# ksahlin/NGSpeciesID

Measured on AMD Instinct MI355X. Metric: reads/sec end-to-end (cluster + spoa consensus + racon x3), 750 bp ONT, higher is better.
Workload: dtype u8 / int16 / int32 DP, 64-bit bit-vectors (f64 thresholds)

## Files before the change

### ngspeciesid_amd/csrc/k_poa.h

```cpp
#pragma once
#include "ngsid_internal.h"

struct PSeq { const uint8_t* s; const uint8_t* q; int32_t len, uw; uint32_t cw; int32_t mode, a0, a1; };

#define POA_MODE_SUBGRAPH 3

struct PoaJobSet {
    const PSeq* seqs; const PSeq* bbs; const uint32_t* seq_idx; const uint32_t* job_off; const int32_t* job_bb; uint32_t njobs; const uint32_t* job_list; uint32_t nrun;
    const uint8_t* job_final;
    const uint32_t* nrun_dev;
    int m, n, g, Vcap, Ecap, Lmax, D, node_cap, trim_tiles;
    int32_t* Hglob; uint8_t* dirglob; uint32_t* covglob;
    uint8_t* out; int32_t* out_len; int32_t* out_span ; uint64_t* out_cw; uint32_t* out_n; uint32_t* out_cov; uint32_t* dropped; uint32_t* slot_overflow; unsigned long long* phase_cycles; int phase_detail; unsigned long long* stat_rows ;
};

__host__ __device__ inline uint32_t poa_ntiles(uint32_t n, uint32_t D) { if (n == 0) return 0; if (D == 0 || n <= D) return 1; const uint32_t r = n % D; return (r != 0 && r < (D + 1) / 2) ? n / D : (n + D - 1) / D; }

struct PoaPlan { int Vcap, Ecap, Lmax; uint32_t nwg_main, nwg_redo; int band0; bool sub = false; };
int32_t poa_check_limits(ngsid_ctx* ctx, const PoaPlan& P, int m, int g);
int32_t poa_prepare(ngsid_ctx* ctx, PoaPlan& P, uint32_t max_jobs, int m, int g);
int32_t poa_launch(ngsid_ctx* ctx, const PoaPlan& P, PoaJobSet J, int band, bool redo, uint32_t* work_ctr, bool sub = false);
```

### ngspeciesid_amd/csrc/ngsid_api.hip

```cpp
#include "ngsid_internal.h"
#include "../../include/ngsid_merge_schedule.h"
#include "../../include/ngsid_tables.h"
#include <math.h>
#include <algorithm>

extern "C" uint32_t ngsid_abi_version(void) { return 2u; }

static char g_static_err[256] = "";
extern "C" const char* ngsid_last_error(ngsid_ctx* ctx) { return ctx ? ctx->err : g_static_err; }

namespace {
struct DevPool { std::mutex mu; std::multimap<unsigned long long, void*> free_; size_t cached = 0; int contexts = 0; size_t live = 0, peak = 0;
                 struct Upload { size_t bs; void* q; size_t bq; void* off; size_t bo; }; std::map<void*, Upload> uploads;
};
DevPool g_pool;
const size_t POOL_LIMIT = (size_t)48 << 30;
const size_t POOL_HEADROOM = (size_t)3 << 30;
struct PoolBlocks { void* p[3] = {nullptr, nullptr, nullptr}; size_t b[3] = {0, 0, 0}; bool owned = true; ~PoolBlocks() { if (owned) for (int i = 0; i < 3; ++i) if (p[i]) ngsid_pool_free(p[i], b[i]); } };
inline size_t pool_class(size_t b) { if (b < 4096) return 4096; int sh = 63 - __builtin_clzll((unsigned long long)b) - 3; size_t m = ((size_t)1 << sh) - 1; return (b + m) & ~m; }
inline unsigned long long pool_key(int dev, size_t cls) { return ((unsigned long long)dev << 56) | (unsigned long long)cls; }
}
thread_local ngsid_ctx* g_ngsid_tls_ctx = nullptr;
hipError_t ngsid_pool_alloc(void** p, size_t bytes, size_t* got)
{
    const size_t cls = pool_class(bytes ? bytes : 1); int dev = 0; (void)hipGetDevice(&dev);
    {
        std::lock_guard<std::mutex> lk(g_pool.mu);
        auto it = g_pool.free_.find(pool_key(dev, cls));
        if (it != g_pool.free_.end()) { *p = it->second; g_pool.free_.erase(it); g_pool.cached -= cls; *got = cls; g_pool.live += cls; g_pool.peak = std::max(g_pool.peak, g_pool.live); return hipSuccess; }
    }
    hipError_t e = hipErrorOutOfMemory;
    for (int attempt = 0; attempt < 2; ++attempt) {
        size_t freeb = 0, totalb = 0;
        const bool known = hipMemGetInfo(&freeb, &totalb) == hipSuccess;
        if (!known || freeb >= cls + std::min<size_t>(POOL_HEADROOM, totalb / 16)) { e = hipMalloc(p, cls); if (e == hipSuccess) break; (void)hipGetLastError(); }
        if (attempt == 0) ngsid_pool_release_all();
    }
    *got = e == hipSuccess ? cls : 0;
    if (e == hipSuccess) { std::lock_guard<std::mutex> lk(g_pool.mu); g_pool.live += cls; g_pool.peak = std::max(g_pool.peak, g_pool.live); }
    return e;
}
void ngsid_pool_free(void* p, size_t bytes)
{
    if (!p) return;
    if (ngsid_ctx* c = g_ngsid_tls_ctx) {
        (void)hipStreamSynchronize(c->stream);
        if (c->ev_fork) for (int i = 0; i < 4; ++i) if (c->side[i]) (void)hipStreamSynchronize(c->side[i]);
    } else (void)hipDeviceSynchronize();
    int dev = 0; (void)hipGetDevice(&dev);
    {
        std::lock_guard<std::mutex> lk(g_pool.mu);
        g_pool.live -= std::min(g_pool.live, bytes);
        if (bytes && g_pool.cached + bytes <= POOL_LIMIT) { g_pool.free_.emplace(pool_key(dev, bytes), p); g_pool.cached += bytes; return; }
    }
    (void)hipFree(p);
}
namespace { struct PinPool { std::mutex mu; std::multimap<size_t, void*> free_; size_t cached = 0; }; PinPool g_pin; const size_t PIN_LIMIT = (size_t)4 << 30; }
void* ngsid_pinned_alloc(size_t bytes)
{
    const size_t cls = pool_class(bytes ? bytes : 1);
    {
        std::lock_guard<std::mutex> lk(g_pin.mu);
        auto it = g_pin.free_.find(cls);
        if (it != g_pin.free_.end()) { void* p = it->second; g_pin.free_.erase(it); g_pin.cached -= cls; return p; }
    }
    void* p = nullptr;
    if (hipHostMalloc(&p, cls, hipHostMallocDefault) != hipSuccess) {
        (void)hipGetLastError();
        std::vector<void*> old; { std::lock_guard<std::mutex> lk(g_pin.mu); for (auto& kv : g_pin.free_) old.push_back(kv.second); g_pin.free_.clear(); g_pin.cached = 0; }
        for (void* q : old) (void)hipHostFree(q);
        if (hipHostMalloc(&p, cls, hipHostMallocDefault) != hipSuccess) { (void)hipGetLastError(); return nullptr; }
    }
    return p;
}
void ngsid_pinned_free(void* p, size_t bytes)
{
    if (!p) return;
    const size_t cls = pool_class(bytes ? bytes : 1);
    {
        std::lock_guard<std::mutex> lk(g_pin.mu);
        if (g_pin.cached + cls <= PIN_LIMIT) { g_pin.free_.emplace(cls, p); g_pin.cached += cls; return; }
    }
    (void)hipHostFree(p);
}
size_t ngsid_pool_cached_bytes() { std::lock_guard<std::mutex> lk(g_pool.mu); return g_pool.cached; }
int ngsid_pool_contexts() { std::lock_guard<std::mutex> lk(g_pool.mu); return g_pool.contexts > 0 ? g_pool.contexts : 1; }
void ngsid_pool_stats(size_t* live, size_t* peak, bool reset_peak) { std::lock_guard<std::mutex> lk(g_pool.mu); if (live) *live = g_pool.live; if (peak) *peak = g_pool.peak; if (reset_peak) g_pool.peak = g_pool.live; }
void ngsid_pool_release_all()
{
    std::lock_guard<std::mutex> lk(g_pool.mu);
    for (auto& kv : g_pool.free_) (void)hipFree(kv.second);
    g_pool.free_.clear(); g_pool.cached = 0;
}

extern "C" int32_t ngsid_create(int32_t device_ordinal, uint32_t flags, ngsid_ctx** out)
{
    (void)flags;
    if (!out) return NGSID_ERR_ARG;
    *out = nullptr;
    int ndev = 0;
    hipError_t e = hipGetDeviceCount(&ndev);
    if (e != hipSuccess || ndev <= 0) { snprintf(g_static_err, sizeof g_static_err, "no HIP device (%s); this library has no CPU path", hipGetErrorString(e)); return NGSID_ERR_NO_DEVICE; }
    if (device_ordinal < 0 || device_ordinal >= ndev) { snprintf(g_static_err, sizeof g_static_err, "device ordinal %d out of range (0..%d)", device_ordinal, ndev - 1); return NGSID_ERR_ARG; }
    e = hipSetDevice(device_ordinal);
    if (e != hipSuccess) { snprintf(g_static_err, sizeof g_static_err, "hipSetDevice: %s", hipGetErrorString(e)); return NGSID_ERR_HIP; }
    ngsid_ctx* c = new ngsid_ctx();
    c->device = device_ordinal;
    c->debug_sync = getenv("NGSID_DEBUG_SYNC") != nullptr;
    hipDeviceProp_t prop;
    if (hipGetDeviceProperties(&prop, device_ordinal) == hipSuccess) {
        c->n_cu = prop.multiProcessorCount > 0 ? prop.multiProcessorCount : 256;
        size_t freeb = 0, totalb = 0;
        if (hipMemGetInfo(&freeb, &totalb) == hipSuccess && freeb > ((size_t)8 << 30)) c->scratch_budget = std::min<size_t>(freeb / 4, (size_t)32 << 30);
    }
    e = hipStreamCreateWithFlags(&c->stream, hipStreamNonBlocking);
    if (e != hipSuccess) { snprintf(g_static_err, sizeof g_static_err, "hipStreamCreate: %s", hipGetErrorString(e)); delete c; return NGSID_ERR_HIP; }
    { std::lock_guard<std::mutex> lk(g_pool.mu); g_pool.contexts++; }
    *out = c;
    return NGSID_OK;
}

extern "C" void ngsid_destroy(ngsid_ctx* ctx)
{
    if (!ctx) return;
    if (g_ngsid_tls_ctx == ctx) g_ngsid_tls_ctx = nullptr;
    (void)hipSetDevice(ctx->device);
    for (int i = 0; i < 4; ++i) { if (ctx->side[i]) { (void)hipStreamSynchronize(ctx->side[i]); (void)hipStreamDestroy(ctx->side[i]); } if (ctx->ev_join[i]) (void)hipEventDestroy(ctx->ev_join[i]); }
    if (ctx->ev_fork) (void)hipEventDestroy(ctx->ev_fork);
    if (ctx->pin) (void)hipHostFree(ctx->pin);
    if (ctx->stream) { (void)hipStreamSynchronize(ctx->stream); (void)hipStreamDestroy(ctx->stream); }
    delete ctx;
    bool last; { std::lock_guard<std::mutex> lk(g_pool.mu); last = --g_pool.contexts <= 0; }
    if (last) {
        {
            std::lock_guard<std::mutex> lk(g_pool.mu);
            for (auto& kv : g_pool.uploads) { (void)hipFree(kv.first); if (kv.second.q) (void)hipFree(kv.second.q); (void)hipFree(kv.second.off); }
            g_pool.uploads.clear();
        }
        ngsid_pool_release_all();
        std::vector<void*> pins; { std::lock_guard<std::mutex> lk(g_pin.mu); for (auto& kv : g_pin.free_) pins.push_back(kv.second); g_pin.free_.clear(); g_pin.cached = 0; }
        for (void* q : pins) (void)hipHostFree(q);
    }
}

int32_t ngsid_side_streams(ngsid_ctx* ctx)
{
    if (ctx->ev_fork) return NGSID_OK;
    for (int i = 0; i < 4; ++i) { HIPCHK(ctx, hipStreamCreateWithFlags(&ctx->side[i], hipStreamNonBlocking)); HIPCHK(ctx, hipEventCreateWithFlags(&ctx->ev_join[i], hipEventDisableTiming)); }
    HIPCHK(ctx, hipEventCreateWithFlags(&ctx->ev_fork, hipEventDisableTiming));
    return NGSID_OK;
}

__global__ __launch_bounds__(256) void k_off_fingerprint(const uint64_t* __restrict__ off, uint64_t n, unsigned long long* __restrict__ out)
{
    unsigned long long h = 0;
    for (uint64_t i = (uint64_t)blockIdx.x * 256 + threadIdx.x; i <= n; i += (uint64_t)gridDim.x * 256) { unsigned long long x = off[i] + (i + 1) * 0xD6E8FEB86659FD93ull; x ^= x >> 31; x *= 0x9E3779B97F4A7C15ull; x ^= x >> 29; h += x; }
#pragma unroll
    for (int d = 32; d >= 1; d >>= 1) h += __shfl_xor(h, d);
    if ((threadIdx.x & 63) == 0) atomicAdd(out, h);
}

int32_t ngsid_upload_reads(ngsid_ctx* ctx, const ngsid_reads_t* in, DevReads* out, bool need_qual)
{
    if (!in || (!in->off) || (in->n && !in->seq)) NGSID_FAIL(ctx, NGSID_ERR_ARG, "null read set");
    if (need_qual && in->n && !in->qual) NGSID_FAIL(ctx, NGSID_ERR_ARG, "this entry point needs qualities");
    HIPCHK(ctx, hipSetDevice(ctx->device));
    HostTimer hu(ctx->stream, "upload_reads");
    out->n = in->n;
    if (in->mem == NGSID_MEM_DEVICE) {
        out->seq = in->seq; out->qual = in->qual; out->off = in->off;
        unsigned long long fp = 0;
        {
            if (ctx->mzc_fp.n < 2) HIPCHK(ctx, ctx->mzc_fp.alloc(2));
            HIPCHK(ctx, hipMemsetAsync(ctx->mzc_fp.p + 1, 0, sizeof(unsigned long long), ctx->stream));
            hipLaunchKernelGGL(k_off_fingerprint, dim3(256), dim3(256), 0, ctx->stream, in->off, in->n, ctx->mzc_fp.p + 1);
            HIPCHK(ctx, hipGetLastError());
            HIPCHK(ctx, hipMemcpyAsync(&fp, ctx->mzc_fp.p + 1, sizeof fp, hipMemcpyDeviceToHost, ctx->stream));
            HIPCHK(ctx, hipStreamSynchronize(ctx->stream));
        }
        if (ctx->offc.v && ctx->offc.ptr == (const void*)in->off && ctx->offc.n == in->n && ctx->offc.fp == fp && ctx->offc.v->size() == in->n + 1) {
            out->h_off.v = ctx->offc.v; out->total = (*out->h_off.v)[in->n]; out->maxlen = ctx->offc.maxlen; out->minlen = ctx->offc.minlen;
            hu.mark("offsets: cached");
            return NGSID_OK;
        }
        out->h_off.resize(in->n + 1);
        hu.mark("resize");
        const size_t nb = sizeof(uint64_t) * (in->n + 1);
        if (ctx->pin_bytes < nb) { if (ctx->pin) (void)hipHostFree(ctx->pin); ctx->pin = nullptr; ctx->pin_bytes = 0; HIPCHK(ctx, hipHostMalloc(&ctx->pin, nb + nb / 8, hipHostMallocDefault)); ctx->pin_bytes = nb + nb / 8; }
        HIPCHK(ctx, hipMemcpyAsync(ctx->pin, in->off, nb, hipMemcpyDeviceToHost, ctx->stream));
        HIPCHK(ctx, hipStreamSynchronize(ctx->stream));
        hu.mark("d2h");
        memcpy(out->h_off.data(), ctx->pin, nb);
        hu.mark("memcpy");
        ctx->offc.ptr = in->off; ctx->offc.n = in->n; ctx->offc.fp = fp; ctx->offc.v = out->h_off.v; ctx->offc.maxlen = 0;
    } else {
        out->h_off.resize(in->n + 1);
        memcpy(out->h_off.data(), in->off, sizeof(uint64_t) * (in->n + 1));
        const uint64_t total = out->h_off[in->n];
        HIPCHK(ctx, out->own_seq.alloc(total + 16)); HIPCHK(ctx, out->own_off.alloc(in->n + 1));
        if (total) HIPCHK(ctx, hipMemcpyAsync(out->own_seq.p, in->seq, total, hipMemcpyHostToDevice, ctx->stream));
        HIPCHK(ctx, hipMemcpyAsync(out->own_off.p, in->off, sizeof(uint64_t) * (in->n + 1), hipMemcpyHostToDevice, ctx->stream));
        out->seq = out->own_seq.p; out->off = out->own_off.p; out->qual = nullptr;
        if (in->qual) { HIPCHK(ctx, out->own_qual.alloc(total + 16)); if (total) HIPCHK(ctx, hipMemcpyAsync(out->own_qual.p, in->qual, total, hipMemcpyHostToDevice, ctx->stream)); out->qual = out->own_qual.p; }
        HIPCHK(ctx, hipStreamSynchronize(ctx->stream));
    }
    out->total = out->h_off[in->n];
    uint32_t mx = 0, mn = 0xffffffffu;
    for (uint64_t i = 0; i < in->n; ++i) {
        if (out->h_off[i + 1] < out->h_off[i]) NGSID_FAIL(ctx, NGSID_ERR_ARG, "offsets not monotone at read %llu", (unsigned long long)i);
        const uint64_t l = out->h_off[i + 1] - out->h_off[i];
        if (l > 0xffffffffull) NGSID_FAIL(ctx, NGSID_ERR_TOO_LONG, "read %llu too long", (unsigned long long)i);
        mx = std::max<uint32_t>(mx, (uint32_t)l); mn = std::min<uint32_t>(mn, (uint32_t)l);
    }
    out->maxlen = mx; out->minlen = in->n ? mn : 0;
    if (in->mem == NGSID_MEM_DEVICE && ctx->offc.v == out->h_off.v) { ctx->offc.maxlen = out->maxlen; ctx->offc.minlen = out->minlen; }
    hu.mark("scan");
    return NGSID_OK;
}

extern "C" int32_t ngsid_sg_align_cigar_batch(ngsid_ctx* ctx, const ngsid_reads_t* queries, const ngsid_reads_t* targets,
                                              const uint32_t* q_idx, const uint32_t* t_idx, uint64_t n_pairs,
                                              int32_t match, int32_t mismatch, const int32_t* open, int32_t ext,
                                              int32_t* score, uint64_t* ops_off, uint8_t* ops, uint64_t cap, uint64_t* needed)
{
    if (!ctx) return NGSID_ERR_ARG;
    if (!queries || !targets || !ops_off || (n_pairs && (!q_idx || !t_idx || !open))) NGSID_FAIL(ctx, NGSID_ERR_ARG, "null argument");
    DevReads Q, T;
    int32_t rc = ngsid_upload_reads(ctx, queries, &Q, false); if (rc) return rc;
    rc = ngsid_upload_reads(ctx, targets, &T, false); if (rc) return rc;
    ops_off[0] = 0;
    if (n_pairs == 0) { if (needed) *needed = 0; return NGSID_OK; }
    uint32_t mq = 0, mt = 0;
    std::vector<uint64_t> h_off(n_pairs + 1, 0);
    for (uint64_t p = 0; p < n_pairs; ++p) {
        if (q_idx[p] >= Q.n || t_idx[p] >= T.n) NGSID_FAIL(ctx, NGSID_ERR_ARG, "pair %llu out of range", (unsigned long long)p);
        const uint32_t ql = (uint32_t)(Q.h_off[q_idx[p] + 1] - Q.h_off[q_idx[p]]), tl = (uint32_t)(T.h_off[t_idx[p] + 1] - T.h_off[t_idx[p]]);
        mq = std::max(mq, ql); mt = std::max(mt, tl);
        h_off[p + 1] = h_off[p] + ql + tl;
    }
    DevBuf<uint32_t> dq, dt; DevBuf<int32_t> dopen, dout; DevBuf<uint64_t> doff; DevBuf<uint8_t> dops;
    HIPCHK(ctx, dq.alloc(n_pairs)); HIPCHK(ctx, dt.alloc(n_pairs)); HIPCHK(ctx, dopen.alloc(n_pairs)); HIPCHK(ctx, dout.alloc(n_pairs * 4)); HIPCHK(ctx, doff.alloc(n_pairs + 1)); HIPCHK(ctx, dops.alloc(h_off[n_pairs] + 1));
    HIPCHK(ctx, hipMemcpyAsync(dq.p, q_idx, 4 * n_pairs, hipMemcpyHostToDevice, ctx->stream));
    HIPCHK(ctx, hipMemcpyAsync(dt.p, t_idx, 4 * n_pairs, hipMemcpyHostToDevice, ctx->stream));
    HIPCHK(ctx, hipMemcpyAsync(dopen.p, open, 4 * n_pairs, hipMemcpyHostToDevice, ctx->stream));
    HIPCHK(ctx, hipMemcpyAsync(doff.p, h_off.data(), 8 * (n_pairs + 1), hipMemcpyHostToDevice, ctx->stream));
    AlignJob J{};
    J.qseq = Q.seq; J.qoff = Q.off; J.tseq = T.seq; J.toff = T.off; J.qidx = dq.p; J.tidx = dt.p; J.npairs = n_pairs;
    J.match = match; J.mismatch = mismatch; J.ext = ext; J.k = 1; J.open = dopen.p; J.match_id = nullptr;
    J.score = dout.p; J.ncols = dout.p + n_pairs; J.nmatch = nullptr; J.region = nullptr; J.bp = nullptr; J.bp_windows = 0; J.window = 1; J.span = nullptr;
    J.ops = dops.p; J.ops_off = doff.p;
    int mo = 0; for (uint64_t p = 0; p < n_pairs; ++p) { if (open[p] < 0) { mo = 1 << 20; break; } mo = std::max(mo, (int)open[p]); }
    rc = ngsid_launch_align(ctx, J, mq, mt, mo); if (rc) return rc;
    std::vector<int32_t> h(n_pairs * 2); std::vector<uint8_t> hops(h_off[n_pairs] + 1);
    HIPCHK(ctx, hipMemcpyAsync(h.data(), dout.p, 8 * n_pairs, hipMemcpyDeviceToHost, ctx->stream));
    HIPCHK(ctx, hipMemcpyAsync(hops.data(), dops.p, h_off[n_pairs], hipMemcpyDeviceToHost, ctx->stream));
    HIPCHK(ctx, hipStreamSynchronize(ctx->stream));
    if (score) memcpy(score, h.data(), 4 * n_pairs);
    uint64_t total = 0; for (uint64_t p = 0; p < n_pairs; ++p) { total += (uint64_t)h[n_pairs + p]; ops_off[p + 1] = total; }
    if (needed) *needed = total;
    if (total > cap || (!ops && total)) NGSID_FAIL(ctx, NGSID_ERR_CAPACITY, "ops buffer too small: need %llu bytes", (unsigned long long)total);
    static const uint8_t sym[4] = {'=', 'X', 'I', 'D'};
    for (uint64_t p = 0; p < n_pairs; ++p) {
        const uint64_t c = (uint64_t)h[n_pairs + p]; const uint8_t* src = hops.data() + h_off[p]; uint8_t* dst = ops + ops_off[p];
        const uint64_t ql = Q.h_off[q_idx[p] + 1] - Q.h_off[q_idx[p]], tl = T.h_off[t_idx[p] + 1] - T.h_off[t_idx[p]];
        if (ql == 0 || tl == 0) { for (uint64_t x = 0; x < c; ++x) dst[x] = ql ? 'I' : 'D'; continue; }
        for (uint64_t x = 0; x < c; ++x) dst[x] = sym[src[c - 1 - x] & 3];
    }
    return NGSID_OK;
}

extern "C" int32_t ngsid_sg_align_batch(ngsid_ctx* ctx, const ngsid_reads_t* queries, const ngsid_reads_t* targets,
                                        const uint32_t* q_idx, const uint32_t* t_idx, uint64_t n_pairs,
                                        int32_t match, int32_t mismatch, const int32_t* open, int32_t ext,
                                        int32_t k, const int32_t* match_id,
                                        int32_t* score, int32_t* n_cols, int32_t* n_match, int32_t* region)
{
    ApiClock api_clock_(ctx, "sg_align_batch");
    if (!ctx) return NGSID_ERR_ARG;
    if (!queries || !targets || (n_pairs && (!q_idx || !t_idx || !open))) NGSID_FAIL(ctx, NGSID_ERR_ARG, "null argument");
    DevReads Q, T;
    int32_t rc = ngsid_upload_reads(ctx, queries, &Q, false); if (rc) return rc;
    rc = ngsid_upload_reads(ctx, targets, &T, false); if (rc) return rc;
    if (n_pairs == 0) return NGSID_OK;
    uint32_t mq = 0, mt = 0;
    for (uint64_t p = 0; p < n_pairs; ++p) {
        if (q_idx[p] >= Q.n || t_idx[p] >= T.n) NGSID_FAIL(ctx, NGSID_ERR_ARG, "pair %llu out of range", (unsigned long long)p);
        mq = std::max<uint32_t>(mq, (uint32_t)(Q.h_off[q_idx[p] + 1] - Q.h_off[q_idx[p]]));
        mt = std::max<uint32_t>(mt, (uint32_t)(T.h_off[t_idx[p] + 1] - T.h_off[t_idx[p]]));
    }
    DevBuf<uint32_t> dq, dt; DevBuf<int32_t> dopen, dmid, dout;
    HIPCHK(ctx, dq.alloc(n_pairs)); HIPCHK(ctx, dt.alloc(n_pairs)); HIPCHK(ctx, dopen.alloc(n_pairs)); HIPCHK(ctx, dmid.alloc(n_pairs)); HIPCHK(ctx, dout.alloc(n_pairs * 4));
    HIPCHK(ctx, hipMemcpyAsync(dq.p, q_idx, 4 * n_pairs, hipMemcpyHostToDevice, ctx->stream));
    HIPCHK(ctx, hipMemcpyAsync(dt.p, t_idx, 4 * n_pairs, hipMemcpyHostToDevice, ctx->stream));
    HIPCHK(ctx, hipMemcpyAsync(dopen.p, open, 4 * n_pairs, hipMemcpyHostToDevice, ctx->stream));
    if (match_id) HIPCHK(ctx, hipMemcpyAsync(dmid.p, match_id, 4 * n_pairs, hipMemcpyHostToDevice, ctx->stream));
    AlignJob J{};
    J.qseq = Q.seq; J.qoff = Q.off; J.tseq = T.seq; J.toff = T.off; J.qidx = dq.p; J.tidx = dt.p; J.npairs = n_pairs;
    J.match = match; J.mismatch = mismatch; J.ext = ext; J.k = k; J.open = dopen.p; J.match_id = match_id ? dmid.p : nullptr;
    J.score = dout.p; J.ncols = dout.p + n_pairs; J.nmatch = dout.p + 2 * n_pairs; J.region = dout.p + 3 * n_pairs;
    J.bp = nullptr; J.bp_windows = 0; J.window = 1; J.span = nullptr;
    int mo = 0; for (uint64_t p = 0; p < n_pairs; ++p) { if (open[p] < 0) { mo = 1 << 20; break; } mo = std::max(mo, (int)open[p]); }
    rc = ngsid_launch_align(ctx, J, mq, mt, mo); if (rc) return rc;
    std::vector<int32_t> h(n_pairs * 4);
    HIPCHK(ctx, hipMemcpyAsync(h.data(), dout.p, 16 * n_pairs, hipMemcpyDeviceToHost, ctx->stream));
    HIPCHK(ctx, hipStreamSynchronize(ctx->stream));
    if (score) memcpy(score, h.data(), 4 * n_pairs);
    if (n_cols) memcpy(n_cols, h.data() + n_pairs, 4 * n_pairs);
    if (n_match) memcpy(n_match, h.data() + 2 * n_pairs, 4 * n_pairs);
    if (region) memcpy(region, h.data() + 3 * n_pairs, 4 * n_pairs);
    return NGSID_OK;
}

extern "C" int32_t ngsid_ed_align_batch(ngsid_ctx* ctx, const ngsid_reads_t* queries, const ngsid_reads_t* targets,
                                        const uint32_t* q_idx, const uint32_t* t_idx, uint64_t n_pairs,
                                        int32_t window, int32_t bp_windows, int32_t* distance, int32_t* span, int32_t* bp)
{
    if (!ctx) return NGSID_ERR_ARG;
    if (!queries || !targets || (n_pairs && (!q_idx || !t_idx))) NGSID_FAIL(ctx, NGSID_ERR_ARG, "null argument");
    if (bp && (bp_windows <= 0 || window <= 0)) NGSID_FAIL(ctx, NGSID_ERR_ARG, "bp needs window > 0 and bp_windows > 0");
    DevReads Q, T;
    int32_t rc = ngsid_upload_reads(ctx, queries, &Q, false); if (rc) return rc;
    rc = ngsid_upload_reads(ctx, targets, &T, false); if (rc) return rc;
    if (n_pairs == 0) return NGSID_OK;
    uint32_t mq = 0, mt = 0;
    for (uint64_t p = 0; p < n_pairs; ++p) {
        if (q_idx[p] >= Q.n || t_idx[p] >= T.n) NGSID_FAIL(ctx, NGSID_ERR_ARG, "pair %llu out of range", (unsigned long long)p);
        mq = std::max<uint32_t>(mq, (uint32_t)(Q.h_off[q_idx[p] + 1] - Q.h_off[q_idx[p]]));
        mt = std::max<uint32_t>(mt, (uint32_t)(T.h_off[t_idx[p] + 1] - T.h_off[t_idx[p]]));
    }
    DevBuf<uint32_t> dq, dt; DevBuf<int32_t> ddist, dspan, dbp;
    HIPCHK(ctx, dq.alloc(n_pairs)); HIPCHK(ctx, dt.alloc(n_pairs)); HIPCHK(ctx, ddist.alloc(n_pairs)); HIPCHK(ctx, dspan.alloc(n_pairs * 4));
    if (bp) HIPCHK(ctx, dbp.alloc(n_pairs * (uint64_t)bp_windows * 4));
    HIPCHK(ctx, hipMemcpyAsync(dq.p, q_idx, 4 * n_pairs, hipMemcpyHostToDevice, ctx->stream));
    HIPCHK(ctx, hipMemcpyAsync(dt.p, t_idx, 4 * n_pairs, hipMemcpyHostToDevice, ctx->stream));
    AlignJob J{};
    J.qseq = Q.seq; J.qoff = Q.off; J.tseq = T.seq; J.toff = T.off; J.qidx = dq.p; J.tidx = dt.p; J.npairs = n_pairs;
    J.bp = bp ? dbp.p : nullptr; J.bp_windows = bp ? bp_windows : 0; J.window = window; J.span = dspan.p;
    rc = ngsid_launch_ed_align(ctx, J, mq, mt, ddist.p); if (rc) return rc;
    if (distance) HIPCHK(ctx, hipMemcpyAsync(distance, ddist.p, 4 * n_pairs, hipMemcpyDeviceToHost, ctx->stream));
    if (span) HIPCHK(ctx, hipMemcpyAsync(span, dspan.p, 16 * n_pairs, hipMemcpyDeviceToHost, ctx->stream));
    if (bp) HIPCHK(ctx, hipMemcpyAsync(bp, dbp.p, 16ull * n_pairs * bp_windows, hipMemcpyDeviceToHost, ctx->stream));
    HIPCHK(ctx, hipStreamSynchronize(ctx->stream));
    return NGSID_OK;
}

extern "C" int32_t ngsid_hpc_minimizers(ngsid_ctx* ctx, const ngsid_reads_t* reads, int32_t k, int32_t w,
                                        uint64_t* mz_off, uint64_t* codes, uint32_t* pos, uint64_t cap, uint64_t* needed,
                                        uint32_t* hpc_len, double* hpc_err)
{
    if (!ctx) return NGSID_ERR_ARG;
    if (!reads || !mz_off) NGSID_FAIL(ctx, NGSID_ERR_ARG, "null argument");
    DevReads R; int32_t rc = ngsid_upload_reads(ctx, reads, &R, false); if (rc) return rc;
    const uint64_t n = R.n;
    DevBuf<uint64_t> ccode, coff; DevBuf<uint32_t> cpos, dcnt, dhl; DevBuf<double> dherr, draw; PinVec<uint64_t> hmoff; PinVec<uint32_t> hcnt(n), hhl(n);
    HIPCHK(ctx, dcnt.alloc(n)); HIPCHK(ctx, dhl.alloc(n)); HIPCHK(ctx, dherr.alloc(n)); HIPCHK(ctx, draw.alloc(n));
    long long bad = -1;
    rc = ngsid_minimizers_csr(ctx, R, k, w, MzOut{&ccode, &cpos, &coff, &hmoff}, dcnt.p, dhl.p, dherr.p, draw.p, hcnt.data(), hhl.data(), &bad); if (rc) return rc;
    if (bad >= 0) NGSID_FAIL(ctx, NGSID_ERR_ALPHABET, "read %lld: base outside ACGTN", bad);
    std::vector<double> hherr(n);
    if (n) HIPCHK(ctx, hipMemcpyAsync(hherr.data(), dherr.p, 8 * n, hipMemcpyDeviceToHost, ctx->stream));
    HIPCHK(ctx, hipStreamSynchronize(ctx->stream));
    const uint64_t total = hmoff[n];
    if (needed) *needed = total;
    if (hpc_len) memcpy(hpc_len, hhl.data(), 4 * n);
    if (hpc_err) memcpy(hpc_err, hherr.data(), 8 * n);
    const bool dev_out = reads->mem == NGSID_MEM_DEVICE;
    if (total > cap || (total && (!codes || !pos))) {
        if (!dev_out) memcpy(mz_off, hmoff.data(), 8 * (n + 1));
        NGSID_FAIL(ctx, NGSID_ERR_CAPACITY, "minimizer buffer too small: need %llu entries", (unsigned long long)total);
    }
    const hipMemcpyKind kind = dev_out ? hipMemcpyDeviceToDevice : hipMemcpyDeviceToHost;
    if (dev_out) HIPCHK(ctx, hipMemcpyAsync(mz_off, coff.p, 8 * (n + 1), kind, ctx->stream)); else memcpy(mz_off, hmoff.data(), 8 * (n + 1));
    if (total) { HIPCHK(ctx, hipMemcpyAsync(codes, ccode.p, 8 * total, kind, ctx->stream)); HIPCHK(ctx, hipMemcpyAsync(pos, cpos.p, 4 * total, kind, ctx->stream)); }
    HIPCHK(ctx, hipStreamSynchronize(ctx->stream));
    return NGSID_OK;
}

__constant__ double c_p_clamped[128];
__constant__ double c_p_nomin[128];
static bool g_score_tables[16] = {false};

#define SC_QS 132
#define SC_SS 68
template <typename HT>
__global__ __launch_bounds__(64)
void k_score_reads(const uint8_t* __restrict__ seq, const uint8_t* __restrict__ qual, const uint64_t* __restrict__ off, uint64_t n,
                   int k, double qthr, double* __restrict__ score, double* __restrict__ err, uint8_t* __restrict__ keep)
{
    __shared__ __attribute__((aligned(16))) uint8_t qt[64 * SC_QS];
    __shared__ __attribute__((aligned(16))) uint8_t st[64 * SC_SS];
    __shared__ HT hist[128 * 64];
    __shared__ double tp[128], tn[128];
    const int lane = threadIdx.x;
    const uint64_t r = (uint64_t)blockIdx.x * 64 + lane;
    const bool have = r < n;
    const uint64_t b = have ? off[r] : 0; const int len = have ? (int)(off[r + 1] - b) : 0;
    tp[lane] = c_p_clamped[lane]; tp[lane + 64] = c_p_clamped[lane + 64]; tn[lane] = c_p_nomin[lane]; tn[lane + 64] = c_p_nomin[lane + 64];
    for (int c = 0; c < 128; ++c) hist[c * 64 + lane] = 0;
    int maxlen = len;
#pragma unroll
    for (int d = 32; d >= 1; d >>= 1) maxlen = max(maxlen, __shfl_xor(maxlen, d));
    maxlen = __builtin_amdgcn_readfirstlane(maxlen);
    const bool active = have && len >= 2 * k;
    int hl = 0; uint8_t prevc = 0;
    double cur = 1.0, sum = 0.0;
    const int sub = lane >> 4, dj = lane & 15;
    for (int c0 = 0; c0 < maxlen; c0 += 64) {
        const int half = c0 & 64;
        for (int it = 0; it < 16; ++it) {
            const int rr = it * 4 + sub;
            const uint64_t rb = __shfl((unsigned long long)b, rr); const int rl = __shfl(len, rr);
            const int x = c0 + dj * 4;
            unsigned qw = 0, sw = 0;
            if (x + 3 < rl) { qw = *(const unsigned*)(qual + rb + x); sw = *(const unsigned*)(seq + rb + x); }
            else for (int y = 0; y < 4; ++y) if (x + y < rl) { qw |= (unsigned)qual[rb + x + y] << (8 * y); sw |= (unsigned)seq[rb + x + y] << (8 * y); }
            *(unsigned*)(qt + rr * SC_QS + half + dj * 4) = qw;
            *(unsigned*)(st + rr * SC_SS + dj * 4) = sw;
        }
        __syncthreads();
        if (active) {
            const int e = min(64, len - c0);
            for (int i = 0; i < e; ++i) {
                const int gi = c0 + i;
                const uint8_t sc = st[lane * SC_SS + i], qc = qt[lane * SC_QS + half + i] & 127;
                hl += (gi == 0 || sc != prevc); prevc = sc;
                hist[qc * 64 + lane] += 1;
                const double pn = 1.0 - tp[qc];
                if (gi < k) { cur = cur * pn; if (gi == k - 1) sum = cur; }
                else { const double leave = 1.0 - tp[qt[lane * SC_QS + ((gi - k) & 127)] & 127]; cur *= (pn / leave); sum += cur; }
            }
        }
        __syncthreads();
    }
    if (!have) return;
    score[r] = 0.0; err[r] = 0.0; keep[r] = 0;
    if (!active || hl < k) return;
    const double ee = (double)(len - k + 1) - sum;
    const double pno = 1.0 - ee / (double)(len - k + 1);
    score[r] = pno * (double)(len - k + 1);
    double se = 0.0;
    for (int c = 0; c < 128; ++c) { const int h = hist[c * 64 + lane]; if (h) se = se + (double)h * tn[c]; }
    const double er = se / (double)len;
    err[r] = er;
    if (10.0 * -(log(er) / log(10.0)) <= qthr) return;
    keep[r] = 1;
}

extern "C" int32_t ngsid_score_reads(ngsid_ctx* ctx, const ngsid_reads_t* reads, int32_t k, double q_threshold,
                                     double* score, double* err_rate, uint8_t* keep)
{
    if (!ctx) return NGSID_ERR_ARG;
    if (!reads || !score || !err_rate || !keep || k < 1) NGSID_FAIL(ctx, NGSID_ERR_ARG, "null argument");
    if (k > 64) NGSID_FAIL(ctx, NGSID_ERR_ARG, "score_reads: k = %d exceeds 64 (the quality ring of the kernel)", (int)k);
    DevReads R; int32_t rc = ngsid_upload_reads(ctx, reads, &R, true); if (rc) return rc;
    if (!g_score_tables[ctx->device & 15]) {
        HIPCHK(ctx, hipMemcpyToSymbol(HIP_SYMBOL(c_p_clamped), NGSID_PHRED_P, sizeof(double) * 128));
        HIPCHK(ctx, hipMemcpyToSymbol(HIP_SYMBOL(c_p_nomin), NGSID_PHRED_P_NOMIN, sizeof(double) * 128));
        g_score_tables[ctx->device & 15] = true;
    }
    const uint64_t n = R.n; if (!n) return NGSID_OK;
    DevBuf<double> ds, de; DevBuf<uint8_t> dk;
    HIPCHK(ctx, ds.alloc(n)); HIPCHK(ctx, de.alloc(n)); HIPCHK(ctx, dk.alloc(n));
    { ProfScope ps_(ctx, "k_score_reads");
      if (R.maxlen <= 65535u) hipLaunchKernelGGL(k_score_reads<unsigned short>, dim3((unsigned)((n + 63) / 64)), dim3(64), 0, ctx->stream, R.seq, R.qual, R.off, n, k, q_threshold, ds.p, de.p, dk.p);
      else hipLaunchKernelGGL(k_score_reads<unsigned int>, dim3((unsigned)((n + 63) / 64)), dim3(64), 0, ctx->stream, R.seq, R.qual, R.off, n, k, q_threshold, ds.p, de.p, dk.p); }
    HIPCHK(ctx, hipGetLastError());
    HIPCHK(ctx, hipMemcpyAsync(score, ds.p, 8 * n, hipMemcpyDeviceToHost, ctx->stream));
    HIPCHK(ctx, hipMemcpyAsync(err_rate, de.p, 8 * n, hipMemcpyDeviceToHost, ctx->stream));
    HIPCHK(ctx, hipMemcpyAsync(keep, dk.p, n, hipMemcpyDeviceToHost, ctx->stream));
    HIPCHK(ctx, hipStreamSynchronize(ctx->stream));
    return NGSID_OK;
}

static void prof_collect(ngsid_ctx* ctx)
{
    (void)hipStreamSynchronize(ctx->stream);
    for (auto& e : ctx->prof_events) {
        float ms = 0.f;
        if (hipEventElapsedTime(&ms, e.a, e.b) == hipSuccess) { auto& acc = ctx->prof_acc[e.name]; acc.first += ms; acc.second += 1; }
        (void)hipEventDestroy(e.a); (void)hipEventDestroy(e.b);
    }
    ctx->prof_events.clear();
}
extern "C" int32_t ngsid_profile_enable(ngsid_ctx* ctx, int32_t on)
{
    if (!ctx) return NGSID_ERR_ARG;
    prof_collect(ctx); ctx->prof_acc.clear(); ctx->prof = on != 0;
    if (on) { if (ctx->stat.n < 8) HIPCHK(ctx, ctx->stat.alloc(8)); HIPCHK(ctx, hipMemsetAsync(ctx->stat.p, 0, 8 * sizeof(unsigned long long), ctx->stream)); HIPCHK(ctx, hipStreamSynchronize(ctx->stream)); }
    return NGSID_OK;
}
extern "C" int32_t ngsid_reads_upload(ngsid_ctx* ctx, const ngsid_reads_t* host, ngsid_reads_t* dev)
{
    if (!ctx) return NGSID_ERR_ARG;
    if (!host || !dev || !host->off || (host->n && !host->seq) || host->mem != NGSID_MEM_HOST) NGSID_FAIL(ctx, NGSID_ERR_ARG, "reads_upload: a host read set and an output are required");
    HIPCHK(ctx, hipSetDevice(ctx->device));
    const uint64_t n = host->n, total = host->off[n];
    PoolBlocks PB; void *&ds = PB.p[0], *&dq = PB.p[1], *&dof = PB.p[2]; size_t &bs = PB.b[0], &bq = PB.b[1], &bo = PB.b[2];
    HIPCHK(ctx, ngsid_pool_alloc(&ds, total + 16, &bs));
    HIPCHK(ctx, ngsid_pool_alloc(&dof, sizeof(uint64_t) * (n + 1), &bo));
    if (host->qual) HIPCHK(ctx, ngsid_pool_alloc(&dq, total + 16, &bq));
    if (total) HIPCHK(ctx, hipMemcpyAsync(ds, host->seq, total, hipMemcpyHostToDevice, ctx->stream));
    if (total && host->qual) HIPCHK(ctx, hipMemcpyAsync(dq, host->qual, total, hipMemcpyHostToDevice, ctx->stream));
    HIPCHK(ctx, hipMemcpyAsync(dof, host->off, sizeof(uint64_t) * (n + 1), hipMemcpyHostToDevice, ctx->stream));
    HIPCHK(ctx, hipStreamSynchronize(ctx->stream));
    { std::lock_guard<std::mutex> lk(g_pool.mu); g_pool.uploads[ds] = {bs, dq, bq, dof, bo}; }
    PB.owned = false;
    dev->seq = (const uint8_t*)ds; dev->qual = (const uint8_t*)dq; dev->off = (const uint64_t*)dof; dev->n = n; dev->mem = NGSID_MEM_DEVICE; dev->_pad = 0;
    return NGSID_OK;
}


__global__ __launch_bounds__(256) void k_reads_subset(const uint8_t* __restrict__ seq, const uint8_t* __restrict__ qual, const uint64_t* __restrict__ off, const uint64_t* __restrict__ idx,
                                                      const uint64_t* __restrict__ noff, uint64_t n, uint8_t* __restrict__ oseq, uint8_t* __restrict__ oqual, unsigned long long* __restrict__ foreign)
{
    const int lane = threadIdx.x & 63;
    const uint64_t r = (uint64_t)blockIdx.x * 4 + (threadIdx.x >> 6);
    if (r >= n) return;
    const uint64_t src = off[idx[r]], dst = noff[r]; const uint64_t len = noff[r + 1] - dst;
    unsigned bad = 0;
    for (uint64_t x = lane; x < len; x += 64) {
        const uint8_t c = seq[src + x]; oseq[dst + x] = c; if (oqual) oqual[dst + x] = qual[src + x];
        bad += !(c == 'A' || c == 'C' || c == 'G' || c == 'T' || c == 'N');
    }
    if (foreign) {
#pragma unroll
        for (int d = 32; d >= 1; d >>= 1) bad += __shfl_xor(bad, d);
        if (lane == 0 && bad) atomicAdd(foreign, (unsigned long long)bad);
    }
}
extern "C" int32_t ngsid_reads_subset(ngsid_ctx* ctx, const ngsid_reads_t* dev_in, const uint64_t* idx, uint64_t n, ngsid_reads_t* dev_out, uint64_t* foreign)
{
    if (!ctx) return NGSID_ERR_ARG;
    ApiClock api_clock_(ctx, "reads_subset");
    if (!dev_in || !dev_out || (n && !idx) || dev_in->mem != NGSID_MEM_DEVICE) NGSID_FAIL(ctx, NGSID_ERR_ARG, "reads_subset: a device read set, an index list and an output are required");
    DevReads R; int32_t rc = ngsid_upload_reads(ctx, dev_in, &R, false); if (rc) return rc;
    static thread_local PinVec<uint64_t> h_noff; h_noff.resize(n + 1); h_noff[0] = 0;
    for (uint64_t i = 0; i < n; ++i) { if (idx[i] >= R.n) NGSID_FAIL(ctx, NGSID_ERR_ARG, "reads_subset: index %llu out of range", (unsigned long long)idx[i]); h_noff[i + 1] = h_noff[i] + (R.h_off[idx[i] + 1] - R.h_off[idx[i]]); }
    const uint64_t total = h_noff[n];
    PoolBlocks PB; void *&ds = PB.p[0], *&dq = PB.p[1], *&dof = PB.p[2]; size_t &bs = PB.b[0], &bq = PB.b[1], &bo = PB.b[2];
    HIPCHK(ctx, ngsid_pool_alloc(&ds, total + 16, &bs));
    HIPCHK(ctx, ngsid_pool_alloc(&dof, sizeof(uint64_t) * (n + 1), &bo));
    if (dev_in->qual) HIPCHK(ctx, ngsid_pool_alloc(&dq, total + 16, &bq));
    DevBuf<uint64_t> d_idx; DevBuf<unsigned long long> d_bad; HIPCHK(ctx, d_idx.alloc(n)); HIPCHK(ctx, d_bad.alloc(1));
    HIPCHK(ctx, hipMemsetAsync(d_bad.p, 0, sizeof(unsigned long long), ctx->stream));
    HIPCHK(ctx, hipMemcpyAsync(dof, h_noff.data(), sizeof(uint64_t) * (n + 1), hipMemcpyHostToDevice, ctx->stream));
    if (n) HIPCHK(ctx, hipMemcpyAsync(d_idx.p, idx, sizeof(uint64_t) * n, hipMemcpyHostToDevice, ctx->stream));
    if (n) hipLaunchKernelGGL(k_reads_subset, dim3((unsigned)((n + 3) / 4)), dim3(256), 0, ctx->stream, R.seq, R.qual, R.off, d_idx.p, (const uint64_t*)dof, n, (uint8_t*)ds, (uint8_t*)dq, d_bad.p);
    HIPCHK(ctx, hipGetLastError());
    unsigned long long hb = 0;
    HIPCHK(ctx, hipMemcpyAsync(&hb, d_bad.p, sizeof hb, hipMemcpyDeviceToHost, ctx->stream));
    HIPCHK(ctx, hipStreamSynchronize(ctx->stream));
    if (foreign) *foreign = hb;
    { std::lock_guard<std::mutex> lk(g_pool.mu); g_pool.uploads[ds] = {bs, dq, bq, dof, bo}; }
    PB.owned = false;
    dev_out->seq = (const uint8_t*)ds; dev_out->qual = (const uint8_t*)dq; dev_out->off = (const uint64_t*)dof; dev_out->n = n; dev_out->mem = NGSID_MEM_DEVICE; dev_out->_pad = 0;
    return NGSID_OK;
}

extern "C" int32_t ngsid_reads_release(ngsid_ctx* ctx, ngsid_reads_t* dev)
{
    if (!ctx) return NGSID_ERR_ARG;
    ApiClock api_clock_(ctx, "reads_release");
    if (!dev || dev->mem != NGSID_MEM_DEVICE) NGSID_FAIL(ctx, NGSID_ERR_ARG, "reads_release: not a device read set");
    DevPool::Upload u;
    { std::lock_guard<std::mutex> lk(g_pool.mu); auto it = g_pool.uploads.find((void*)dev->seq); if (it == g_pool.uploads.end()) NGSID_FAIL(ctx, NGSID_ERR_ARG, "reads_release: this read set was not made by ngsid_reads_upload (or was released already)"); u = it->second; g_pool.uploads.erase(it); }
    ngsid_pool_free((void*)dev->seq, u.bs); if (u.q) ngsid_pool_free(u.q, u.bq); ngsid_pool_free(u.off, u.bo);
    dev->seq = nullptr; dev->qual = nullptr; dev->off = nullptr; dev->n = 0;
    return NGSID_OK;
}

extern "C" int32_t ngsid_ctx_option(ngsid_ctx* ctx, const char* name, int64_t value)
{
    if (!ctx || !name) return NGSID_ERR_ARG;
    static const char* known[] = {"minimizers_chunk_bases", "poa_level_budget_mb", "cluster_block", "cluster_block_cap", "cluster_trunc", "cluster_seg_order", "ed_band", "ed_win_all", "align32", "align_noclass", "poa_tiles_per_cu", "minimizers_lean", "minimizers_mode", "poa_host_levels", "align_paired", "poa_out_slots", "ed_lds_pad_kb", "ed_win6", "support_budget_mb", "demux_chunk_reads"};
    for (const char* k : known) if (!strcmp(k, name)) { ctx->options[name] = (long long)value; return NGSID_OK; }
    if (!strcmp(name, "touch")) {
        if (ctx->mzc_fp.n < 2) HIPCHK(ctx, ctx->mzc_fp.alloc(2));
        HIPCHK(ctx, hipMemsetAsync(ctx->mzc_fp.p + 1, 0, sizeof(unsigned long long), ctx->stream)); HIPCHK(ctx, hipStreamSynchronize(ctx->stream));
        return NGSID_OK;
    }
    if (!strcmp(name, "release_scratch")) {
        (void)hipStreamSynchronize(ctx->stream);
        ctx->tb.release(); ctx->bnd.release(); ctx->tb_long.release(); ctx->bnd_long.release(); ctx->aln_cls.release(); ctx->aln_psorted.release(); ctx->aln_pbin.release(); ctx->ed_tb.release(); ctx->ed_h.release(); ctx->ed_fail.release(); ctx->ed_fail2.release();
        ctx->poa_h.release(); ctx->poa_d.release(); ctx->poa_g.release(); ctx->poa_cov.release();
        for (auto& L : ctx->poa_lv) { L.out.release(); L.seqs.release(); L.job_final.release(); L.out_len.release(); L.out_span.release(); L.job_bb.release(); L.out_cw.release(); L.out_n.release(); L.out_cov.release(); L.job_off.release(); L.seq_idx.release(); L.flags.release(); L.job_list.release(); L.job_unit.release(); L.job_pos.release(); }
        ctx->mzc.valid = false; ctx->mzc_cnt.release(); ctx->mzc_hlen.release(); ctx->mz_off.release(); ctx->mz_scode.release(); ctx->mz_spos.release();
        ctx->pol_mzcode.release(); ctx->pol_mzpos.release(); ctx->pol_oseq.release(); ctx->pol_oqual.release(); ctx->pol_valid.release(); ctx->pol_bp.release(); ctx->pol_lay.release(); ctx->cl_cnt.release();
        ngsid_pool_release_all();
        return NGSID_OK;
    }
    if (!strcmp(name, "scratch_budget_mb")) {
        if (value < 64) NGSID_FAIL(ctx, NGSID_ERR_ARG, "scratch_budget_mb must be at least 64");
        ctx->scratch_budget = (size_t)value << 20; return NGSID_OK;
    }
    NGSID_FAIL(ctx, NGSID_ERR_ARG, "unknown option '%s'", name);
}

extern "C" int32_t ngsid_profile_read(ngsid_ctx* ctx, char* buf, uint64_t cap)
{
    if (!ctx || !buf || !cap) return NGSID_ERR_ARG;
    prof_collect(ctx);
    std::string out;
    for (auto& kv : ctx->prof_acc) { char line[256]; snprintf(line, sizeof line, "%s %llu %.6f\n", kv.first.c_str(), (unsigned long long)kv.second.second, kv.second.first); out += line; }
    ctx->prof_acc.clear();
    { char line[128]; snprintf(line, sizeof line, "poa_band_redo_tiles %llu 0.0\n", (unsigned long long)ctx->poa_redo_tiles); out += line; ctx->poa_redo_tiles = 0; }
    {
        size_t live = 0, peak = 0; ngsid_pool_stats(&live, &peak, true);
        char line[160]; snprintf(line, sizeof line, "hbm_live_bytes %llu 0.0\nhbm_peak_bytes %llu 0.0\n", (unsigned long long)live, (unsigned long long)peak); out += line;
        size_t lv = 0; for (auto& L : ctx->poa_lv) lv += L.out.abytes + L.seqs.abytes + L.out_len.abytes + L.out_span.abytes + L.job_bb.abytes + L.out_cw.abytes + L.out_n.abytes + L.out_cov.abytes + L.job_off.abytes + L.seq_idx.abytes + L.job_list.abytes + L.job_unit.abytes + L.job_pos.abytes;
        const struct { const char* nm; size_t b; } parts[] = {
            {"mem_cluster_aligner_traceback", ctx->tb.abytes + ctx->bnd.abytes + ctx->tb_long.abytes + ctx->bnd_long.abytes + ctx->aln_cls.abytes + ctx->aln_psorted.abytes + ctx->aln_pbin.abytes + ctx->aln_pint.abytes},
            {"mem_polish_aligner_traceback", ctx->ed_tb.abytes + ctx->ed_h.abytes + ctx->ed_fail.abytes + ctx->ed_fail2.abytes},
            {"mem_poa_resident_tiles", ctx->poa_h.abytes + ctx->poa_d.abytes + ctx->poa_g.abytes + ctx->poa_cov.abytes},
            {"mem_poa_level_buffers", lv},
            {"mem_minimizers_compact", ctx->pol_mzcode.abytes + ctx->pol_mzpos.abytes + ctx->mz_off.abytes + ctx->mzc_cnt.abytes + ctx->mzc_hlen.abytes},
            {"mem_minimizers_sparse_chunk", ctx->mz_scode.abytes + ctx->mz_spos.abytes},
            {"mem_oriented_reads", ctx->pol_oseq.abytes + ctx->pol_oqual.abytes},
            {"mem_cluster_hit_matrix", ctx->cl_cnt.abytes},
            {"mem_polish_layers", ctx->pol_valid.abytes + ctx->pol_bp.abytes + ctx->pol_lay.abytes}};
        for (const auto& pt : parts) { snprintf(line, sizeof line, "%s %llu 0.0\n", pt.nm, (unsigned long long)pt.b); out += line; }
    }
    if (ctx->stat.p) {
        unsigned long long h[8] = {0}; HIPCHK(ctx, hipMemcpy(h, ctx->stat.p, sizeof h, hipMemcpyDeviceToHost)); HIPCHK(ctx, hipMemset(ctx->stat.p, 0, sizeof h));
        char line[160]; snprintf(line, sizeof line, "poa_dp_rows %llu 0.0\nsg_dp_cells %llu 0.0\n", h[0], h[1]); out += line;
    }
    if (out.size() + 1 > cap) NGSID_FAIL(ctx, NGSID_ERR_CAPACITY, "profile buffer too small");
    memcpy(buf, out.c_str(), out.size() + 1);
    return NGSID_OK;
}

static int32_t merge_cb(void* user, const ngsid_reads_t* sub, const ngsid_cluster_params_t* prm, const uint32_t* acc_rank, const int32_t* prev_batch, const double* known_err,
                        int32_t* rep_of_read, double* hpc_err_out, uint8_t* status_out)
{
    uint64_t counters[4];
    return ngsid_cluster_greedy((ngsid_ctx*)user, sub, prm, acc_rank, prev_batch, known_err, rep_of_read, hpc_err_out, status_out, counters);
}
extern "C" int32_t ngsid_merge_representatives(ngsid_ctx* ctx, const ngsid_reads_t* reps, const ngsid_cluster_params_t* prm, const uint32_t* acc_rank,
                                               const double* score, const double* hpc_err, const int32_t* batch, int32_t n_batches, int32_t* rep_of)
{
    if (!ctx) return NGSID_ERR_ARG;
    if (!reps || !prm || !rep_of || (reps->n && (!score || !batch))) NGSID_FAIL(ctx, NGSID_ERR_ARG, "null argument");
    if (reps->mem != NGSID_MEM_HOST || (reps->n && !reps->qual)) NGSID_FAIL(ctx, NGSID_ERR_ARG, "representatives are expected as a host read set with qualities (they are a few KB each)");
    return ngsid_merge_schedule(merge_cb, ctx, reps, prm, acc_rank, score, hpc_err, batch, n_batches, rep_of);
}
```

### ngspeciesid_amd/csrc/poa_host.hip

```cpp
#include "ngsid_internal.h"
#include "k_poa.h"
#include <thread>
#include <atomic>
#include <chrono>
#include <algorithm>
#include <vector>
#include <string>
#include <memory>

namespace {

struct Unit {
    std::vector<uint32_t> seqs;
    int bb = -1;
    bool done = false;
    uint32_t single_maxlen = 0;
    std::string result; std::vector<uint32_t> cov; bool has_result = false;
};

__host__ __device__ inline int32_t poa_base_weight(uint64_t w) { return w > (1u << 20) ? (1 << 20) : w < 1 ? 1 : (int32_t)w; }

__host__ __device__ inline PSeq poa_tile_pseq(const uint8_t* s, uint64_t cw, int32_t len, int mode, int bb, const int32_t& wlen, const int32_t* span)
{
    PSeq S; S.s = s; S.q = nullptr; S.len = len; S.uw = poa_base_weight(cw); S.cw = (uint32_t)(cw > 0xffffffffull ? 0xffffffffull : cw); S.mode = mode; S.a0 = 0; S.a1 = -1;
    if (bb >= 0) {
        const int offset = (int)(0.01 * (double)wlen), begin = span[0], end = span[1];
        if (end >= begin) { S.a0 = begin; S.a1 = end; S.mode = (begin < offset && end > wlen - offset) ? NGSID_POA_GLOBAL : NGSID_POA_SEMI; }
    }
    return S;
}

__global__ void k_make_pseq_reads(const uint8_t* seq, const uint8_t* qual, const uint64_t* off, uint64_t n, int mode, const uint32_t* weight, PSeq* out)
{
    const uint64_t i = (uint64_t)blockIdx.x * blockDim.x + threadIdx.x;
    if (i >= n) return;
    PSeq S; S.s = seq + off[i]; S.q = qual ? qual + off[i] : nullptr; S.len = (int32_t)(off[i + 1] - off[i]); S.uw = 1; S.cw = 1; S.mode = mode; S.a0 = 0; S.a1 = -1;
    if (weight) {
        const uint32_t wv = weight[i]; S.q = nullptr; S.cw = wv; S.uw = poa_base_weight(wv);
    }
    out[i] = S;
}

struct HierParams { int m, n, g, band, node_cap, D, upper_mode; bool want_cov; int trim_tiles; int single_below = 0; bool sub = false; };

struct TileLists {
    PinVec<uint32_t> job_off, seq_idx, job_unit; PinVec<int32_t> job_bb; PinVec<uint8_t> job_final ;
    uint32_t maxD, maxn; int maxbb; bool any_nobb;
    uint32_t njobs() const { return (uint32_t)job_unit.size(); }
};
void build_tiles(TileLists& T, std::vector<Unit>& units, const std::vector<int>& bb_len, int D, uint32_t* unit_rec)
{
    T.job_off.assign(1, 0); T.seq_idx.clear(); T.job_unit.clear(); T.job_bb.clear(); T.job_final.clear();
    T.maxD = 0; T.maxn = 0; T.maxbb = 0; T.any_nobb = false;
    { size_t tot = 0; for (const Unit& U : units) if (!U.done) tot += U.seqs.size(); T.seq_idx.reserve(tot); }
    const size_t nu = units.size();
    for (size_t u = 0; u < nu; ++u) {
        Unit& U = units[u];
        const uint32_t ncur = U.done ? 0u : (uint32_t)U.seqs.size(), job0 = T.njobs();
        if (ncur == 0) U.done = true;
        else {
            const uint32_t Dl = D > 0 ? (uint32_t)D : ncur, nt = poa_ntiles(ncur, Dl), base = (uint32_t)T.seq_idx.size();
            T.seq_idx.insert(T.seq_idx.end(), U.seqs.begin(), U.seqs.end());
            for (uint32_t t = 0; t < nt; ++t) {
                const uint32_t a = t * Dl, b = t + 1 == nt ? ncur : a + Dl;
                T.job_off.push_back(base + b); T.job_bb.push_back(U.bb); T.job_unit.push_back((uint32_t)u); T.job_final.push_back(nt == 1 ? 1 : 0);
                T.maxD = std::max(T.maxD, b - a);
            }
            if (U.bb >= 0) T.maxbb = std::max(T.maxbb, bb_len[U.bb]); else T.any_nobb = true;
            T.maxn = std::max(T.maxn, ncur);
        }
        if (unit_rec) { unit_rec[u] = ncur; unit_rec[nu + u] = job0; unit_rec[2 * nu + u] = T.njobs() - job0; }
    }
}
int32_t upload_tiles(ngsid_ctx* ctx, const TileLists& T, ngsid_ctx::PoaLevelBufs& B, bool final_, bool unit)
{
    HIPCHK(ctx, B.job_off.reserve(T.job_off.size())); HIPCHK(ctx, B.seq_idx.reserve(T.seq_idx.size())); HIPCHK(ctx, B.job_bb.reserve(T.job_bb.size()));
    HIPCHK(ctx, hipMemcpyAsync(B.job_off.p, T.job_off.data(), 4 * T.job_off.size(), hipMemcpyHostToDevice, ctx->stream));
    HIPCHK(ctx, hipMemcpyAsync(B.seq_idx.p, T.seq_idx.data(), 4 * T.seq_idx.size(), hipMemcpyHostToDevice, ctx->stream));
    HIPCHK(ctx, hipMemcpyAsync(B.job_bb.p, T.job_bb.data(), 4 * T.job_bb.size(), hipMemcpyHostToDevice, ctx->stream));
    if (final_) { HIPCHK(ctx, B.job_final.reserve(T.job_final.size())); HIPCHK(ctx, hipMemcpyAsync(B.job_final.p, T.job_final.data(), T.job_final.size(), hipMemcpyHostToDevice, ctx->stream)); }
    if (unit) { HIPCHK(ctx, B.job_unit.reserve(T.job_unit.size())); HIPCHK(ctx, hipMemcpyAsync(B.job_unit.p, T.job_unit.data(), 4 * T.job_unit.size(), hipMemcpyHostToDevice, ctx->stream)); }
    return NGSID_OK;
}

PoaPlan poa_plan(const HierParams& hp, int L0, uint32_t Lm, bool sub)
{
    long long capV = (long long)L0 * (hp.node_cap > 0 ? hp.node_cap : 28) / 16; capV = std::max<long long>(capV, L0 + 64); capV = std::max<long long>(capV, (long long)Lm + 1);
    capV = (capV + 7) & ~7ll;
    PoaPlan P{};
    P.Vcap = (int)capV; P.Ecap = (int)(3 * capV / 2); P.Lmax = (int)((std::max<uint32_t>(Lm, 1) + 15) & ~15u);
    P.band0 = hp.band <= 64 ? 64 : (hp.band <= 128 ? 128 : 256); P.sub = sub;
    return P;
}

PoaJobSet level_jobs(ngsid_ctx* ctx, const HierParams& hp, const PoaPlan& P, int level, int slots, const PSeq* seqs, const PSeq* bbs, const uint32_t* seq_idx, uint32_t njobs, uint32_t* flags)
{
    const ngsid_ctx::PoaLevelBufs& B = ctx->poa_lv[level & 1];
    PoaJobSet J{};
    J.seqs = seqs; J.bbs = bbs; J.seq_idx = seq_idx; J.job_off = B.job_off.p; J.job_bb = B.job_bb.p; J.njobs = njobs;
    J.m = hp.m; J.n = hp.n; J.g = hp.g; J.Vcap = P.Vcap; J.Ecap = P.Ecap; J.Lmax = P.Lmax; J.D = slots; J.node_cap = hp.node_cap;
    J.trim_tiles = (hp.trim_tiles & 1) | ((level > 0 && (hp.trim_tiles & 1)) ? 2 : 0); J.job_final = (hp.trim_tiles & 4) ? B.job_final.p : nullptr;
    J.out = B.out.p; J.out_len = B.out_len.p; J.out_cw = B.out_cw.p; J.out_n = B.out_n.p; J.out_cov = (hp.want_cov || hp.trim_tiles) ? B.out_cov.p : nullptr; J.out_span = B.out_span.p;
    J.dropped = flags; J.slot_overflow = flags + 1;
    return J;
}

int32_t run_hierarchy_host(ngsid_ctx* ctx, const PSeq* d_level0, uint32_t maxlen0, const PSeq* d_bbs, const std::vector<int>& bb_len,
                           std::vector<Unit>& units, const HierParams& hp)
{
    const PSeq* cur = d_level0; uint32_t cur_maxlen = maxlen0;
    int slots_cap = 0;
    HostTimer ht(ctx->stream, "hierarchy");
    if (ctx->poa_ctr.n < 1) HIPCHK(ctx, ctx->poa_ctr.alloc(16));
    for (int level = 0;; ++level) {
        static thread_local TileLists T;
        build_tiles(T, units, bb_len, hp.D, nullptr);
        const uint32_t njobs = T.njobs(), maxD = T.maxD;
        if (njobs == 0) break;
        if (level == 0) ht.mark("L0 host job lists");
        PoaPlan plan = poa_plan(hp, std::max({1, T.maxbb, T.any_nobb ? (int)cur_maxlen : 0}), cur_maxlen, hp.sub && level == 0);
        { int32_t rc = poa_prepare(ctx, plan, njobs, hp.m, hp.g); if (rc) return rc; }
        const int capV = plan.Vcap;
        ngsid_ctx::PoaLevelBufs* Lv = &ctx->poa_lv[level & 1];
        DevBuf<uint32_t>& d_flags = Lv->flags;
        { int32_t rc = upload_tiles(ctx, T, *Lv, hp.trim_tiles & 4, false); if (rc) return rc; }
        HIPCHK(ctx, d_flags.reserve(4));
        int slots = slots_cap ? slots_cap : (int)std::min<uint32_t>(maxD, (uint32_t)std::max<long long>(1, ngsid_opt(ctx, "poa_out_slots", 4)));
        static thread_local PinVec<uint32_t> h_out_n; static thread_local PinVec<int32_t> h_out_len, h_out_span; static thread_local PinVec<uint64_t> h_out_cw;
        const bool need_cov = hp.want_cov || hp.trim_tiles;
        auto launch = [&](const PoaJobSet& J, int bw, bool redo) -> int32_t {
            HIPCHK(ctx, hipMemsetAsync(ctx->poa_ctr.p, 0, sizeof(uint32_t), ctx->stream));
            return poa_launch(ctx, plan, J, bw, redo, ctx->poa_ctr.p, plan.sub);
        };
        for (;;) {
            HIPCHK(ctx, Lv->out.reserve((size_t)njobs * slots * capV)); HIPCHK(ctx, Lv->out_len.reserve((size_t)njobs * slots)); HIPCHK(ctx, Lv->out_cw.reserve((size_t)njobs * slots)); HIPCHK(ctx, Lv->out_n.reserve(njobs)); HIPCHK(ctx, Lv->out_span.reserve((size_t)njobs * slots * 2));
            if (need_cov) HIPCHK(ctx, Lv->out_cov.reserve((size_t)njobs * slots * capV));
            HIPCHK(ctx, hipMemsetAsync(d_flags.p, 0, 16, ctx->stream));
            PoaJobSet J = level_jobs(ctx, hp, plan, level, slots, cur, d_bbs, Lv->seq_idx.p, njobs, d_flags.p);
            J.nrun = njobs;
            DevBuf<unsigned long long> d_ph; static const bool want_ph = getenv("NGSID_POA_PHASES") != nullptr;
            if (want_ph) { HIPCHK(ctx, d_ph.alloc(24 * 256)); HIPCHK(ctx, hipMemsetAsync(d_ph.p, 0, 192 * 256, ctx->stream)); J.phase_cycles = d_ph.p; J.phase_detail = atoi(getenv("NGSID_POA_PHASES")) >= 2; }
            if (level == 0) ht.mark("L0 alloc + upload");
            int32_t rc = launch(J, plan.band0, false); if (rc) return rc;
            if (level == 0) ht.mark("L0 kernel");
            uint32_t h_flags[4];
            h_out_n.resize(njobs); h_out_len.resize((size_t)njobs * slots); h_out_cw.resize((size_t)njobs * slots); h_out_span.resize((size_t)njobs * slots * 2);
            auto download = [&]() -> int32_t {
                HIPCHK(ctx, hipMemcpyAsync(h_flags, d_flags.p, 16, hipMemcpyDeviceToHost, ctx->stream));
                HIPCHK(ctx, hipMemcpyAsync(h_out_n.data(), Lv->out_n.p, 4ull * njobs, hipMemcpyDeviceToHost, ctx->stream));
                HIPCHK(ctx, hipMemcpyAsync(h_out_len.data(), Lv->out_len.p, 4ull * njobs * slots, hipMemcpyDeviceToHost, ctx->stream));
                HIPCHK(ctx, hipMemcpyAsync(h_out_cw.data(), Lv->out_cw.p, 8ull * njobs * slots, hipMemcpyDeviceToHost, ctx->stream));
                HIPCHK(ctx, hipMemcpyAsync(h_out_span.data(), Lv->out_span.p, 8ull * njobs * slots, hipMemcpyDeviceToHost, ctx->stream));
                HIPCHK(ctx, hipStreamSynchronize(ctx->stream));
                return NGSID_OK;
            };
            rc = download(); if (rc) return rc;
            for (int bw = plan.band0; bw < 256 && !h_flags[1] && !h_flags[2];) {
                static thread_local PinVec<uint32_t> redo; redo.clear();
                for (uint32_t j = 0; j < njobs; ++j) if (h_out_n[j] & 0x80000000u) redo.push_back(j);
                if (redo.empty()) break;
                bw *= 2;
                HIPCHK(ctx, Lv->job_list.reserve(redo.size()));
                HIPCHK(ctx, hipMemcpyAsync(Lv->job_list.p, redo.data(), 4 * redo.size(), hipMemcpyHostToDevice, ctx->stream));
                J.job_list = Lv->job_list.p; J.nrun = (uint32_t)redo.size();
                rc = launch(J, bw, true); if (rc) return rc;
                rc = download(); if (rc) return rc;
                ctx->poa_redo_tiles += redo.size();
            }
            for (uint32_t j = 0; j < njobs; ++j) h_out_n[j] &= 0x7fffffffu;
            if (want_ph) { std::vector<unsigned long long> hs(24 * 256); HIPCHK(ctx, hipMemcpy(hs.data(), d_ph.p, 192 * 256, hipMemcpyDeviceToHost)); unsigned long long h[24] = {0}; for (int s_ = 0; s_ < 256; ++s_) for (int k_ = 0; k_ < 24; ++k_) h[k_] += hs[s_ * 24 + k_]; fprintf(stderr, "[ngsid poa phases, Mcycles] jobs %u prepass %.1f forward %.1f traceback %.1f update %.1f emit %.1f | rows %llu non-chain %llu | sums: bestv %llu bestpk %llu nnew %llu alnsum %llu outlen %llu | tb iters %llu reloads %llu reload Mcycles %.1f | emit backtrack %.1f | row kinds: tight %llu in %llu runs, chain %llu, near %llu, generic %llu | update: A %.1f S+D %.1f N %.1f\n", njobs, h[0] / 1e6, h[1] / 1e6, h[2] / 1e6, h[3] / 1e6, h[4] / 1e6, h[5], h[6], h[8], h[9], h[10], h[11], h[12], h[7], h[13], h[14] / 1e6, h[15] / 1e6, h[16], h[17], h[18], h[19], h[20], h[21] / 1e6, h[22] / 1e6, h[23] / 1e6); }
            if (h_flags[2]) NGSID_FAIL(ctx, NGSID_ERR_HIP, "internal: POA tile kernel loop guard tripped (code %u)", h_flags[2]);
            if (!h_flags[1]) break;
            if (slots >= (int)maxD) NGSID_FAIL(ctx, NGSID_ERR_HIP, "internal: POA output slot overflow at full depth");
            slots = (int)std::min<uint32_t>(maxD, (uint32_t)slots * 4); slots_cap = slots;
        }
        if (level == 0) ht.mark("L0 download");
        std::vector<std::vector<uint32_t>> outs(units.size());
        for (uint32_t j = 0; j < njobs; ++j) for (uint32_t s = 0; s < h_out_n[j]; ++s) outs[T.job_unit[j]].push_back(j * (uint32_t)slots + s);
        static thread_local PinVec<PSeq> next; uint32_t next_maxlen = 0;
        { size_t tot = 0; for (uint32_t j = 0; j < njobs; ++j) tot += h_out_n[j]; next.clear(); next.reserve(tot); }
        for (size_t u = 0; u < units.size(); ++u) {
            Unit& U = units[u]; if (U.done) continue;
            const std::vector<uint32_t>& O = outs[u];
            const size_t ncur = U.seqs.size();
            int pick = -1;
            if (O.empty()) { U.done = true; continue; }
            if (O.size() == 1) pick = 0;
            else if (O.size() >= ncur) { pick = 0; for (size_t i = 1; i < O.size(); ++i) if (h_out_cw[O[i]] > h_out_cw[O[pick]]) pick = (int)i; }
            if (pick >= 0) {
                const uint32_t sl = O[pick]; const int len = h_out_len[sl];
                U.result.resize(len);
                if (len) HIPCHK(ctx, hipMemcpy(&U.result[0], Lv->out.p + (size_t)sl * capV, len, hipMemcpyDeviceToHost));
                if (hp.want_cov) { U.cov.resize(len); if (len) HIPCHK(ctx, hipMemcpy(U.cov.data(), Lv->out_cov.p + (size_t)sl * capV, 4ull * len, hipMemcpyDeviceToHost)); }
                U.has_result = true; U.done = true; continue;
            }
            U.seqs.clear();
            for (uint32_t sl : O) {
                const PSeq S = poa_tile_pseq(Lv->out.p + (size_t)sl * capV, h_out_cw[sl], h_out_len[sl], hp.upper_mode, U.bb, U.bb >= 0 ? bb_len[U.bb] : 0, &h_out_span[2 * (size_t)sl]);
                U.seqs.push_back((uint32_t)next.size()); next.push_back(S); next_maxlen = std::max<uint32_t>(next_maxlen, (uint32_t)S.len);
            }
        }
        if (level == 0) ht.mark("L0 distribute"); else { char lb[48]; snprintf(lb, sizeof lb, "level %d (%u tiles)", level, njobs); ht.mark(lb); }
        if (next.empty()) break;
        HIPCHK(ctx, Lv->seqs.reserve(sizeof(PSeq) * next.size()));
        HIPCHK(ctx, hipMemcpyAsync(Lv->seqs.p, next.data(), sizeof(PSeq) * next.size(), hipMemcpyHostToDevice, ctx->stream));
        HIPCHK(ctx, hipStreamSynchronize(ctx->stream));
        cur = (const PSeq*)Lv->seqs.p; cur_maxlen = next_maxlen;
    }
    ht.mark("levels >= 1");
    return NGSID_OK;
}


enum { C_NJOBS = 0 , C_NSEQ = 2, C_OVERFLOW = 3, C_RES_USED = 4, C_REDO_TOTAL = 5, C_FLAGS = 8 , C_REDO = 16 , C_MAXLV = 48, C_WORK = C_REDO + 2 * C_MAXLV , C_WORDS = C_WORK + 3 * C_MAXLV };

struct HierDev {
    uint32_t U; int D, slots, capV, upper_mode, want_cov, Lmax, keep_final; uint32_t cap_jobs[2];
    const int32_t* unit_bb; const int32_t* unit_wlen;
    uint32_t* unit_ncur; uint32_t* unit_job0[2]; uint32_t* unit_njobs[2]; uint32_t* unit_seq0; int32_t* unit_pick; uint32_t* unit_tmp ;
    uint32_t* res_off; int32_t* res_len; uint8_t* res; uint32_t* res_cov;
    uint32_t* ctrl;
};
struct LevelDev { PSeq* seqs; uint8_t* out; int32_t* out_len; int32_t* out_span; uint64_t* out_cw; uint32_t* out_n; uint32_t* out_cov; uint32_t* job_off; int32_t* job_bb; uint32_t* job_unit; uint32_t* job_pos; uint32_t* job_list; uint8_t* job_final; };

__global__ __launch_bounds__(256) void k_poa_redo_list(const uint32_t* __restrict__ out_n, const uint32_t* __restrict__ njobs, uint32_t* __restrict__ list, uint32_t* __restrict__ cnt, uint32_t* __restrict__ total)
{
    const uint32_t n = *njobs; const int lane = threadIdx.x & 63;
    for (uint32_t j0 = blockIdx.x * blockDim.x; j0 < n; j0 += gridDim.x * blockDim.x) {
        const uint32_t j = j0 + threadIdx.x;
        const bool f = j < n && (out_n[j] & 0x80000000u);
        const unsigned long long m = __ballot(f);
        if (!m) continue;
        const int leader = __ffsll((long long)m) - 1;
        uint32_t base = 0; if (lane == leader) { base = atomicAdd(cnt, (uint32_t)__popcll(m)); atomicAdd(total, (uint32_t)__popcll(m)); }
        base = __shfl(base, leader);
        if (f) list[base + __popcll(m & ((1ull << lane) - 1))] = j;
    }
}

__device__ __forceinline__ uint32_t block_excl_scan_256(uint32_t v, uint32_t* sm , uint32_t& total)
{
    const int lane = threadIdx.x & 63, w = threadIdx.x >> 6;
    uint32_t x = v;
#pragma unroll
    for (int d = 1; d < 64; d <<= 1) { const uint32_t y = __shfl_up(x, d); if (lane >= d) x += y; }
    __syncthreads();
    if (lane == 63) sm[w] = x;
    __syncthreads();
    uint32_t off = 0; for (int k = 0; k < w; ++k) off += sm[k];
    total = sm[0] + sm[1] + sm[2] + sm[3];
    return off + x - v;
}

__global__ __launch_bounds__(256) void k_poa_unit_scan(HierDev H, LevelDev Lv, int par)
{
    __shared__ uint32_t sm[8]; __shared__ unsigned long long best_s[4]; __shared__ uint32_t one_slot;
    const uint32_t u = blockIdx.x; if (u >= H.U || H.ctrl[C_OVERFLOW]) return;
    const uint32_t j0 = H.unit_job0[par][u], nj = H.unit_njobs[par][u];
    uint32_t* tmp = H.unit_tmp + 3ull * u;
    if (nj == 0) {
        if (threadIdx.x == 0) { if (H.unit_pick[u] == -2) H.unit_pick[u] = -1; else if (H.unit_pick[u] >= 0 || H.unit_pick[u] == -1) H.unit_pick[u] = -3; tmp[0] = 0; tmp[1] = 0; tmp[2] = 0; }
        return;
    }
    if (threadIdx.x == 0) one_slot = 0xffffffffu;
    __syncthreads();
    uint32_t running = 0;
    for (uint32_t b = 0; b < nj; b += 256) {
        const uint32_t x = b + threadIdx.x; const uint32_t j = j0 + x;
        const uint32_t c = x < nj ? (Lv.out_n[j] & 0x7fffffffu) : 0u;
        uint32_t tot; const uint32_t ex = block_excl_scan_256(c, sm, tot);
        if (x < nj) Lv.job_pos[j] = running + ex;
        if (c) one_slot = j * (uint32_t)H.slots;
        running += tot;
        __syncthreads();
    }
    const uint32_t T = running, ncur = H.unit_ncur[u];
    int pick = -2;
    if (T == 0) pick = -1;
    else if (T == 1) { __syncthreads(); pick = (int)one_slot; }
    else if (T >= ncur) {
        unsigned long long best = 0ull;
        uint32_t bslot = 0;
        for (uint32_t x = threadIdx.x; x < nj; x += 256) {
            const uint32_t j = j0 + x; const uint32_t c = Lv.out_n[j] & 0x7fffffffu; const uint32_t pos = Lv.job_pos[j];
            for (uint32_t sidx = 0; sidx < c; ++sidx) {
                unsigned long long cw = Lv.out_cw[(size_t)j * H.slots + sidx]; if (cw > 0xFFFFFFFFFEull) cw = 0xFFFFFFFFFEull;
                const unsigned long long key = ((cw + 1) << 24) | (unsigned long long)(0xFFFFFFu - ((pos + sidx) & 0xFFFFFFu));
                if (key > best) { best = key; bslot = j * (uint32_t)H.slots + sidx; }
            }
        }
        unsigned long long kb = best; uint32_t sb = bslot;
#pragma unroll
        for (int d = 32; d >= 1; d >>= 1) { const unsigned long long ok = __shfl_xor(kb, d); const uint32_t os = __shfl_xor(sb, d); if (ok > kb) { kb = ok; sb = os; } }
        if ((threadIdx.x & 63) == 0) { best_s[threadIdx.x >> 6] = kb; sm[4 + (threadIdx.x >> 6)] = sb; }
        __syncthreads();
        unsigned long long kk = 0ull; uint32_t ss = 0; for (int k = 0; k < 4; ++k) if (best_s[k] > kk) { kk = best_s[k]; ss = sm[4 + k]; }
        pick = (int)ss;
    }
    if (threadIdx.x == 0) {
        H.unit_pick[u] = pick;
        if (pick == -2) { H.unit_ncur[u] = T; tmp[0] = H.D > 0 ? poa_ntiles(T, (uint32_t)H.D) : 1u; tmp[1] = T; tmp[2] = 0; }
        else { tmp[0] = 0; tmp[1] = 0; tmp[2] = pick >= 0 ? (uint32_t)Lv.out_len[pick] : 0u; }
    }
}

__global__ __launch_bounds__(1024) void k_poa_unit_offsets(HierDev H, int par)
{
    __shared__ uint32_t wsum[3][16]; __shared__ uint32_t carry[3];
    const int lane = threadIdx.x & 63, w = threadIdx.x >> 6;
    if (H.ctrl[C_OVERFLOW]) { if (threadIdx.x == 0) H.ctrl[C_NJOBS + (par ^ 1)] = 0; return; }
    if (threadIdx.x < 3) carry[threadIdx.x] = threadIdx.x == 2 ? H.ctrl[C_RES_USED] : 0u;
    __syncthreads();
    for (uint32_t b = 0; b < H.U; b += 1024) {
        const uint32_t u = b + threadIdx.x; uint32_t v[3] = {0, 0, 0};
        if (u < H.U) { v[0] = H.unit_tmp[3ull * u]; v[1] = H.unit_tmp[3ull * u + 1]; v[2] = H.unit_tmp[3ull * u + 2]; }
        uint32_t x[3] = {v[0], v[1], v[2]};
#pragma unroll
        for (int d = 1; d < 64; d <<= 1) for (int k = 0; k < 3; ++k) { const uint32_t y = __shfl_up(x[k], d); if (lane >= d) x[k] += y; }
        if (lane == 63) for (int k = 0; k < 3; ++k) wsum[k][w] = x[k];
        __syncthreads();
        uint32_t off[3], tot[3];
        for (int k = 0; k < 3; ++k) { off[k] = carry[k]; for (int q = 0; q < w; ++q) off[k] += wsum[k][q]; tot[k] = 0; for (int q = 0; q < 16; ++q) tot[k] += wsum[k][q]; }
        if (u < H.U) {
            H.unit_job0[par ^ 1][u] = off[0] + x[0] - v[0]; H.unit_njobs[par ^ 1][u] = v[0];
            H.unit_seq0[u] = off[1] + x[1] - v[1];
            if (H.unit_pick[u] >= 0) H.res_off[u] = off[2] + x[2] - v[2];
        }
        __syncthreads();
        if (threadIdx.x < 3) carry[threadIdx.x] += tot[threadIdx.x];
        __syncthreads();
    }
    if (threadIdx.x == 0) {
        const uint32_t nj = carry[0], ns = carry[1];
        H.unit_job0[par ^ 1][H.U] = nj;
        H.ctrl[C_RES_USED] = carry[2];
        bool ovf = nj > H.cap_jobs[par ^ 1] || ns > H.cap_jobs[par] * (uint32_t)H.slots || H.ctrl[C_OVERFLOW] != 0 || H.ctrl[C_FLAGS + 1] != 0 || H.ctrl[C_FLAGS + 2] != 0;
        if (ovf) H.ctrl[C_OVERFLOW] = 1;
        H.ctrl[C_NJOBS + (par ^ 1)] = ovf ? 0u : nj; H.ctrl[C_NSEQ] = ns;
    }
}

__global__ __launch_bounds__(256) void k_poa_fill_next(HierDev H, LevelDev Lv, int par)
{
    const int lane = threadIdx.x & 63;
    const uint32_t njobs = H.ctrl[C_NJOBS + par];
    if (H.ctrl[C_OVERFLOW]) return;
    for (uint32_t j = blockIdx.x * (blockDim.x >> 6) + (threadIdx.x >> 6); j < njobs; j += gridDim.x * (blockDim.x >> 6)) {
    const uint32_t u = Lv.job_unit[j]; const int pick = H.unit_pick[u];
    const uint32_t n = Lv.out_n[j] & 0x7fffffffu;
    if (pick == -2) {
        if ((uint32_t)lane < n) {
            const size_t sl = (size_t)j * H.slots + lane;
            const PSeq S = poa_tile_pseq(Lv.out + sl * (size_t)H.capV, Lv.out_cw[sl], Lv.out_len[sl], H.upper_mode, H.unit_bb[u], H.unit_wlen[u], Lv.out_span + 2 * sl);
            if (S.len > H.Lmax) atomicExch(&H.ctrl[C_OVERFLOW], 1u);
            Lv.seqs[H.unit_seq0[u] + Lv.job_pos[j] + (uint32_t)lane] = S;
        }
    } else if (pick >= 0 && (uint32_t)pick / (uint32_t)H.slots == j) {
        const int len = Lv.out_len[pick]; const uint8_t* src = Lv.out + (size_t)pick * H.capV; uint8_t* dst = H.res + H.res_off[u];
        for (int x = lane; x < len; x += 64) dst[x] = src[x];
        if (H.want_cov) { const uint32_t* cs = Lv.out_cov + (size_t)pick * H.capV; uint32_t* cd = H.res_cov + H.res_off[u]; for (int x = lane; x < len; x += 64) cd[x] = cs[x]; }
        if (lane == 0) H.res_len[u] = len;
    }
    }
}

__global__ __launch_bounds__(256) void k_poa_fill_jobs(HierDev H, LevelDev Nx, int par )
{
    const uint32_t nj = H.ctrl[C_NJOBS + (par ^ 1)];
    if (H.ctrl[C_OVERFLOW]) return;
    const uint32_t* j0 = H.unit_job0[par ^ 1];
    for (uint32_t t = blockIdx.x * blockDim.x + threadIdx.x; t < nj; t += gridDim.x * blockDim.x) {
    uint32_t lo = 0, hi = H.U;
    while (hi - lo > 1) { const uint32_t mid = (lo + hi) >> 1; if (j0[mid] <= t) lo = mid; else hi = mid; }
    const uint32_t u = lo, tl = t - j0[u];
    const uint32_t T = H.unit_ncur[u]; const uint32_t Dl = H.D > 0 ? (uint32_t)H.D : T;
    Nx.job_off[t] = H.unit_seq0[u] + tl * Dl; Nx.job_bb[t] = H.unit_bb[u]; Nx.job_unit[t] = u;
    if (H.keep_final) Nx.job_final[t] = H.unit_njobs[par ^ 1][u] == 1 ? 1 : 0;
    if (t == nj - 1) Nx.job_off[nj] = H.ctrl[C_NSEQ];
    }
}


int32_t run_hierarchy_dev(ngsid_ctx* ctx, const PSeq* d_level0, uint32_t maxlen0, const PSeq* d_bbs, const std::vector<int>& bb_len,
                          std::vector<Unit>& units, const HierParams& hp, bool* done)
{
    *done = false;
    static const bool want_ph = getenv("NGSID_POA_PHASES") != nullptr;
    if (want_ph || ngsid_opt(ctx, "poa_host_levels", 0) || units.empty()) return NGSID_OK;
    const uint32_t U = (uint32_t)units.size();
    HostTimer ht(ctx->stream, "hierarchy (device levels)");
    static thread_local TileLists T; static thread_local PinVec<uint32_t> u_u32; static thread_local PinVec<int32_t> u_i32;
    u_u32.assign(3ull * U, 0); u_i32.assign(3ull * U, 0);
    build_tiles(T, units, bb_len, hp.D, u_u32.data());
    for (uint32_t u = 0; u < U; ++u) { const int bb = units[u].bb; u_i32[u] = bb; u_i32[U + u] = bb >= 0 ? bb_len[bb] : 0; u_i32[2ull * U + u] = -2; }
    const uint32_t njobs0 = T.njobs(), maxD = T.maxD; const uint64_t maxn = T.maxn;
    if (njobs0 == 0) return NGSID_OK;
    const int Lb = std::max<int>((int)maxlen0, T.maxbb), Lb2 = Lb + Lb / 4 + 16;
    PoaPlan plan = poa_plan(hp, std::max(T.maxbb, T.any_nobb ? Lb2 : 1), (uint32_t)Lb2, hp.sub);
    if (poa_check_limits(nullptr, plan, hp.m, hp.g)) return NGSID_OK;
    const int band0 = plan.band0; const long long capV = plan.Vcap;
    const int slots = (int)std::min<uint32_t>(maxD, (uint32_t)std::max<long long>(1, ngsid_opt(ctx, "poa_out_slots", 4)));
    int levels_est = 0; { uint64_t n = maxn; const uint32_t Dd = hp.D > 0 ? (uint32_t)hp.D : (uint32_t)std::min<uint64_t>(maxn, 0xffffffffull); while (n > 1 && levels_est < C_MAXLV - 4) { n = poa_ntiles((uint32_t)n, std::max<uint32_t>(Dd, 2u)); ++levels_est; } }
    levels_est = std::min(std::max(levels_est, 1), C_MAXLV - 2);
    uint32_t cap[2]; cap[0] = njobs0;
    { const uint64_t e1 = hp.D > 0 ? (njobs0 + (uint64_t)hp.D - 1) / (uint64_t)hp.D * (uint64_t)slots + U : U; cap[1] = (uint32_t)std::min<uint64_t>(njobs0, e1 + e1 / 4 + 1024); }
    { int32_t rc = poa_prepare(ctx, plan, njobs0, hp.m, hp.g); if (rc) return rc; }
    const bool need_cov = hp.want_cov || hp.trim_tiles;
    LevelDev L[2];
    for (int q = 0; q < 2; ++q) {
        ngsid_ctx::PoaLevelBufs* B = &ctx->poa_lv[q]; const size_t ns = (size_t)cap[q] * slots;
        HIPCHK(ctx, B->out.reserve(ns * capV)); HIPCHK(ctx, B->out_len.reserve(ns)); HIPCHK(ctx, B->out_cw.reserve(ns)); HIPCHK(ctx, B->out_span.reserve(ns * 2)); HIPCHK(ctx, B->out_n.reserve(cap[q]));
        if (need_cov) HIPCHK(ctx, B->out_cov.reserve(ns * capV));
        HIPCHK(ctx, B->seqs.reserve(sizeof(PSeq) * ns)); HIPCHK(ctx, B->job_off.reserve((size_t)cap[q] + 1)); HIPCHK(ctx, B->job_bb.reserve(cap[q])); HIPCHK(ctx, B->job_list.reserve(cap[q]));
        HIPCHK(ctx, B->job_unit.reserve(cap[q])); HIPCHK(ctx, B->job_pos.reserve(cap[q])); HIPCHK(ctx, B->job_final.reserve(cap[q]));
        L[q] = LevelDev{(PSeq*)B->seqs.p, B->out.p, B->out_len.p, B->out_span.p, B->out_cw.p, B->out_n.p, need_cov ? B->out_cov.p : nullptr, B->job_off.p, B->job_bb.p, B->job_unit.p, B->job_pos.p, B->job_list.p, B->job_final.p};
    }
    DevBuf<uint32_t> d_u32, d_ctrl, d_res_off, d_res_cov; DevBuf<int32_t> d_i32, d_res_len; DevBuf<uint8_t> d_res;
    HIPCHK(ctx, d_u32.alloc(9ull * U + 4)); HIPCHK(ctx, d_i32.alloc(3ull * U)); HIPCHK(ctx, d_ctrl.alloc(C_WORDS)); HIPCHK(ctx, d_res_off.alloc(U)); HIPCHK(ctx, d_res_len.alloc(U));
    HIPCHK(ctx, d_res.alloc((size_t)U * capV)); if (hp.want_cov) HIPCHK(ctx, d_res_cov.alloc((size_t)U * capV));
    HierDev H{};
    H.U = U; H.D = hp.D; H.slots = slots; H.capV = (int)capV; H.upper_mode = hp.upper_mode; H.want_cov = hp.want_cov ? 1 : 0; H.Lmax = plan.Lmax; H.keep_final = (hp.trim_tiles & 4) ? 1 : 0; H.cap_jobs[0] = cap[0]; H.cap_jobs[1] = cap[1];
    H.unit_bb = d_i32.p; H.unit_wlen = d_i32.p + U; H.unit_pick = d_i32.p + 2ull * U;
    H.unit_ncur = d_u32.p; H.unit_job0[0] = d_u32.p + U; H.unit_njobs[0] = d_u32.p + 2ull * U + 1; H.unit_job0[1] = d_u32.p + 3ull * U + 1; H.unit_njobs[1] = d_u32.p + 4ull * U + 2; H.unit_seq0 = d_u32.p + 5ull * U + 2; H.unit_tmp = d_u32.p + 6ull * U + 2;
    H.res_off = d_res_off.p; H.res_len = d_res_len.p; H.res = d_res.p; H.res_cov = hp.want_cov ? d_res_cov.p : nullptr; H.ctrl = d_ctrl.p;
    HIPCHK(ctx, hipMemsetAsync(d_ctrl.p, 0, sizeof(uint32_t) * C_WORDS, ctx->stream));
    HIPCHK(ctx, hipMemsetAsync(d_res_len.p, 0xff, sizeof(int32_t) * U, ctx->stream));
    HIPCHK(ctx, hipMemcpyAsync(H.unit_ncur, u_u32.data(), 4ull * U, hipMemcpyHostToDevice, ctx->stream));
    HIPCHK(ctx, hipMemcpyAsync(H.unit_job0[0], u_u32.data() + U, 4ull * U, hipMemcpyHostToDevice, ctx->stream));
    HIPCHK(ctx, hipMemcpyAsync(H.unit_njobs[0], u_u32.data() + 2ull * U, 4ull * U, hipMemcpyHostToDevice, ctx->stream));
    HIPCHK(ctx, hipMemcpyAsync(d_i32.p, u_i32.data(), 12ull * U, hipMemcpyHostToDevice, ctx->stream));
    { int32_t rc = upload_tiles(ctx, T, ctx->poa_lv[0], hp.trim_tiles & 4, true); if (rc) return rc; }
    static thread_local PinVec<uint32_t> h_nj; h_nj.assign(1, njobs0);
    HIPCHK(ctx, hipMemcpyAsync(d_ctrl.p + C_NJOBS, h_nj.data(), 4, hipMemcpyHostToDevice, ctx->stream));
    ht.mark("L0 lists + upload");
    static thread_local PinVec<uint32_t> h_ctrl; h_ctrl.resize(C_WORDS);
    int level = 0;
    for (;;) {
        const int batch_end = std::min(C_MAXLV - 1, level + (level == 0 ? levels_est : 3));
        for (; level < batch_end; ++level) {
            const int par = level & 1; LevelDev& Lv = L[par]; LevelDev& Nx = L[par ^ 1];
            PoaJobSet J = level_jobs(ctx, hp, plan, level, slots, level == 0 ? d_level0 : (const PSeq*)Nx.seqs, d_bbs, level == 0 ? ctx->poa_lv[0].seq_idx.p : nullptr, cap[par], d_ctrl.p + C_FLAGS);
            J.nrun_dev = d_ctrl.p + C_NJOBS + par;
            int32_t rc = poa_launch(ctx, plan, J, band0, false, d_ctrl.p + C_WORK + 3 * level, hp.sub && level == 0); if (rc) return rc;
            int stage = 0;
            for (int bw = band0 * 2; bw <= 256; bw *= 2, ++stage) {
                uint32_t* cnt = d_ctrl.p + C_REDO + 2 * level + stage;
                hipLaunchKernelGGL(k_poa_redo_list, dim3(std::min<uint32_t>((cap[par] + 255) / 256, 1024u)), dim3(256), 0, ctx->stream, Lv.out_n, d_ctrl.p + C_NJOBS + par, Lv.job_list, cnt, d_ctrl.p + C_REDO_TOTAL);
                PoaJobSet R = J; R.job_list = Lv.job_list; R.nrun_dev = cnt;
                rc = poa_launch(ctx, plan, R, bw, true, d_ctrl.p + C_WORK + 3 * level + 1 + stage, hp.sub && level == 0); if (rc) return rc;
            }
            hipLaunchKernelGGL(k_poa_unit_scan, dim3(U), dim3(256), 0, ctx->stream, H, Lv, par);
            hipLaunchKernelGGL(k_poa_unit_offsets, dim3(1), dim3(1024), 0, ctx->stream, H, par);
            hipLaunchKernelGGL(k_poa_fill_next, dim3(std::min<uint32_t>((cap[par] + 3) / 4, 4096u)), dim3(256), 0, ctx->stream, H, Lv, par);
            hipLaunchKernelGGL(k_poa_fill_jobs, dim3(std::min<uint32_t>((cap[par ^ 1] + 255) / 256, 1024u)), dim3(256), 0, ctx->stream, H, Nx, par);
            HIPCHK(ctx, hipGetLastError());
        }
        HIPCHK(ctx, hipMemcpyAsync(h_ctrl.data(), d_ctrl.p, 4 * C_WORDS, hipMemcpyDeviceToHost, ctx->stream));
        HIPCHK(ctx, hipStreamSynchronize(ctx->stream));
        if (h_ctrl[C_FLAGS + 2]) NGSID_FAIL(ctx, NGSID_ERR_HIP, "internal: POA tile kernel loop guard tripped (code %u)", h_ctrl[C_FLAGS + 2]);
        if (h_ctrl[C_OVERFLOW] || h_ctrl[C_FLAGS + 1]) { ht.mark("gave up (geometry): host-driven loop"); return NGSID_OK; }
        if (h_ctrl[C_NJOBS + (level & 1)] == 0) break;
        if (level >= C_MAXLV - 1) return NGSID_OK;
    }
    ctx->poa_redo_tiles += h_ctrl[C_REDO_TOTAL];
    ht.mark("levels");
    static thread_local PinVec<int32_t> h_len; static thread_local PinVec<uint32_t> h_off, h_cov; static thread_local PinVec<uint8_t> h_res;
    h_len.resize(U); h_off.resize(U); const size_t used = h_ctrl[C_RES_USED];
    HIPCHK(ctx, hipMemcpyAsync(h_len.data(), d_res_len.p, 4ull * U, hipMemcpyDeviceToHost, ctx->stream));
    HIPCHK(ctx, hipMemcpyAsync(h_off.data(), d_res_off.p, 4ull * U, hipMemcpyDeviceToHost, ctx->stream));
    h_res.resize(used + 1); if (used) HIPCHK(ctx, hipMemcpyAsync(h_res.data(), d_res.p, used, hipMemcpyDeviceToHost, ctx->stream));
    if (hp.want_cov) { h_cov.resize(used + 1); if (used) HIPCHK(ctx, hipMemcpyAsync(h_cov.data(), d_res_cov.p, 4 * used, hipMemcpyDeviceToHost, ctx->stream)); }
    HIPCHK(ctx, hipStreamSynchronize(ctx->stream));
    for (uint32_t u = 0; u < U; ++u) {
        Unit& Un = units[u]; if (Un.done) continue;
        Un.done = true; Un.seqs.clear();
        if (h_len[u] < 0) continue;
        const int len = h_len[u];
        Un.result.assign((const char*)h_res.data() + h_off[u], (size_t)len);
        if (hp.want_cov) Un.cov.assign(h_cov.data() + h_off[u], h_cov.data() + h_off[u] + len);
        Un.has_result = true;
    }
    ht.mark("results");
    *done = true;
    return NGSID_OK;
}

static int32_t run_hierarchy_batch(ngsid_ctx* ctx, const PSeq* d_level0, uint32_t maxlen0, const PSeq* d_bbs, const std::vector<int>& bb_len,
                                   std::vector<Unit>& units, const HierParams& hp)
{
    bool done = false;
    int32_t rc = run_hierarchy_dev(ctx, d_level0, maxlen0, d_bbs, bb_len, units, hp, &done);
    if (rc || done) return rc;
    return run_hierarchy_host(ctx, d_level0, maxlen0, d_bbs, bb_len, units, hp);
}

int32_t run_hierarchy(ngsid_ctx* ctx, const PSeq* d_level0, uint32_t maxlen0, const PSeq* d_bbs, const std::vector<int>& bb_len,
                      std::vector<Unit>& units, const HierParams& hp)
{
    if (hp.single_below > 0) {
        HierParams hb = hp; hb.single_below = 0;
        for (int cls = 0; cls < 2; ++cls) {
            std::vector<size_t> pick; uint32_t mx = 0;
            for (size_t u = 0; u < units.size(); ++u) if (!units[u].done && units[u].single_maxlen > 0 && (units[u].single_maxlen <= NGSID_POA_SINGLE_MAXLEN) == (cls == 0)) { pick.push_back(u); mx = std::max(mx, units[u].single_maxlen); }
            if (pick.empty()) continue;
            HierParams hs = hb; hs.D = 0; if (cls == 0) hs.node_cap = NGSID_POA_SINGLE_NODE_CAP;
            std::vector<Unit> sub; sub.reserve(pick.size());
            for (size_t u : pick) sub.push_back(std::move(units[u]));
            const int32_t rc = run_hierarchy(ctx, d_level0, std::min(maxlen0, mx), d_bbs, bb_len, sub, hs);
            for (size_t x = 0; x < pick.size(); ++x) { units[pick[x]] = std::move(sub[x]); units[pick[x]].done = true; }
            if (rc) return rc;
        }
        bool any = false; for (const Unit& U : units) any = any || !U.done;
        if (!any) return NGSID_OK;
        return run_hierarchy(ctx, d_level0, maxlen0, d_bbs, bb_len, units, hb);
    }
    size_t budget = 0;
    { const long long mb = ngsid_opt(ctx, "poa_level_budget_mb", 0);
      if (mb > 0) budget = (size_t)mb << 20;
      else {
          size_t freeb = 0, totalb = 0; if (hipMemGetInfo(&freeb, &totalb) != hipSuccess) freeb = (size_t)16 << 30;
          size_t own = 0; for (auto& L : ctx->poa_lv) own += L.out.abytes + L.out_cov.abytes + L.seqs.abytes;
          budget = std::min<size_t>(std::max<size_t>((freeb + own + ngsid_pool_cached_bytes()) / (3 * (size_t)ngsid_pool_contexts()), (size_t)1 << 30), (size_t)48 << 30);
      } }
    int maxbb = 0; for (const Unit& U : units) if (!U.done && U.bb >= 0) maxbb = std::max(maxbb, bb_len[U.bb]);
    const int Lb = std::max<int>((int)maxlen0, maxbb), Lb2 = Lb + Lb / 4 + 16;
    long long capV = (long long)Lb2 * (hp.node_cap > 0 ? hp.node_cap : 28) / 16; capV = std::max<long long>(capV, Lb2 + 64);
    const long long slots = std::max<long long>(1, ngsid_opt(ctx, "poa_out_slots", 4));
    const bool need_cov = hp.want_cov || hp.trim_tiles;
    const double per_tile = (double)slots * ((double)capV * (need_cov ? 5.0 : 1.0) + 64.0) * (hp.D > 0 ? 1.0 + 1.25 * (double)slots / (double)hp.D : 1.0) + 32.0;
    std::vector<std::pair<size_t, size_t>> batches; size_t b0 = 0; double acc = 0;
    for (size_t u = 0; u < units.size(); ++u) {
        const uint32_t ncur = units[u].done ? 0u : (uint32_t)units[u].seqs.size();
        const double need = ncur ? per_tile * (double)poa_ntiles(ncur, hp.D > 0 ? (uint32_t)hp.D : ncur) : 0.0;
        if (u > b0 && acc + need > (double)budget) { batches.push_back({b0, u}); b0 = u; acc = 0; }
        acc += need;
    }
    batches.push_back({b0, units.size()});
    if (batches.size() == 1) return run_hierarchy_batch(ctx, d_level0, maxlen0, d_bbs, bb_len, units, hp);
    for (auto& bt : batches) {
        std::vector<Unit> sub; sub.reserve(bt.second - bt.first);
        for (size_t u = bt.first; u < bt.second; ++u) sub.push_back(std::move(units[u]));
        const int32_t rc = run_hierarchy_batch(ctx, d_level0, maxlen0, d_bbs, bb_len, sub, hp);
        for (size_t u = bt.first; u < bt.second; ++u) units[u] = std::move(sub[u - bt.first]);
        if (rc) return rc;
    }
    return NGSID_OK;
}

}

static int32_t poa_consensus_impl(ngsid_ctx* ctx, const ngsid_reads_t* reads, const uint32_t* read_order, const uint64_t* grp_off, uint64_t n_groups,
                                  const ngsid_poa_params_t* prm, uint64_t* cons_off, uint8_t* cons, uint64_t cons_cap, uint64_t* needed, uint32_t* cov, const uint32_t* weight = nullptr);

extern "C" int32_t ngsid_poa_consensus_weighted(ngsid_ctx* ctx, const ngsid_reads_t* reads, const uint32_t* read_order, const uint64_t* grp_off, uint64_t n_groups,
                                                const ngsid_poa_params_t* prm, const uint32_t* weight, uint64_t* cons_off, uint8_t* cons, uint64_t cons_cap, uint64_t* needed)
{
    if (ctx && !weight) NGSID_FAIL(ctx, NGSID_ERR_ARG, "null weight array");
    return poa_consensus_impl(ctx, reads, read_order, grp_off, n_groups, prm, cons_off, cons, cons_cap, needed, nullptr, weight);
}

extern "C" int32_t ngsid_poa_consensus(ngsid_ctx* ctx, const ngsid_reads_t* reads, const uint32_t* read_order, const uint64_t* grp_off, uint64_t n_groups,
                                       const ngsid_poa_params_t* prm, uint64_t* cons_off, uint8_t* cons, uint64_t cons_cap, uint64_t* needed)
{
    ApiClock api_clock_(ctx, "poa_consensus");
    return poa_consensus_impl(ctx, reads, read_order, grp_off, n_groups, prm, cons_off, cons, cons_cap, needed, nullptr);
}

extern "C" int32_t ngsid_poa_consensus_cov(ngsid_ctx* ctx, const ngsid_reads_t* reads, const uint32_t* read_order, const uint64_t* grp_off, uint64_t n_groups,
                                           const ngsid_poa_params_t* prm, uint64_t* cons_off, uint8_t* cons, uint32_t* cov, uint64_t cons_cap, uint64_t* needed)
{
    if (ctx && !cov) NGSID_FAIL(ctx, NGSID_ERR_ARG, "null coverage buffer");
    return poa_consensus_impl(ctx, reads, read_order, grp_off, n_groups, prm, cons_off, cons, cons_cap, needed, cov);
}

static int32_t poa_consensus_impl(ngsid_ctx* ctx, const ngsid_reads_t* reads, const uint32_t* read_order, const uint64_t* grp_off, uint64_t n_groups,
                                  const ngsid_poa_params_t* prm, uint64_t* cons_off, uint8_t* cons, uint64_t cons_cap, uint64_t* needed, uint32_t* cov, const uint32_t* weight)
{
    if (!ctx) return NGSID_ERR_ARG;
    if (!reads || !grp_off || !prm || !cons_off) NGSID_FAIL(ctx, NGSID_ERR_ARG, "null argument");
    HostTimer htc(ctx->stream, "consensus");
    DevReads RD; int32_t rc = ngsid_upload_reads(ctx, reads, &RD, false); if (rc) return rc;
    htc.mark("upload");
    if (!read_order && grp_off[n_groups] > RD.n) NGSID_FAIL(ctx, NGSID_ERR_ARG, "group offsets exceed the read set");
    if (read_order) for (uint64_t x = 0; x < grp_off[n_groups]; ++x) if (read_order[x] >= RD.n) NGSID_FAIL(ctx, NGSID_ERR_ARG, "read_order[%llu] out of range", (unsigned long long)x);
    htc.mark("checks");
    DevBuf<PSeq> d_seqs; HIPCHK(ctx, d_seqs.alloc(RD.n));
    DevBuf<uint32_t> d_weight; if (weight && RD.n) { HIPCHK(ctx, d_weight.alloc(RD.n)); HIPCHK(ctx, hipMemcpyAsync(d_weight.p, weight, 4 * RD.n, hipMemcpyHostToDevice, ctx->stream)); }
    if (RD.n) hipLaunchKernelGGL(k_make_pseq_reads, dim3((unsigned)((RD.n + 255) / 256)), dim3(256), 0, ctx->stream, RD.seq, RD.qual, RD.off, RD.n, prm->mode, weight ? d_weight.p : (const uint32_t*)nullptr, d_seqs.p);
    HIPCHK(ctx, hipGetLastError());
    std::vector<Unit> units(n_groups);
    for (uint64_t g = 0; g < n_groups; ++g) {
        if (read_order) units[g].seqs.assign(read_order + grp_off[g], read_order + grp_off[g + 1]);
        else { units[g].seqs.resize(grp_off[g + 1] - grp_off[g]); for (uint64_t r = grp_off[g]; r < grp_off[g + 1]; ++r) units[g].seqs[r - grp_off[g]] = (uint32_t)r; }
    }
    HierParams hp{prm->match, prm->mismatch, prm->gap, prm->band > 0 ? prm->band : (RD.maxlen <= NGSID_POA_BAND64_MAXLEN ? 64 : 128), prm->node_cap, prm->tile_depth, prm->mode, cov != nullptr, prm->trim > 0 ? 1 : 0};
    hp.single_below = prm->single_below > 0 ? prm->single_below : 0;
    if (hp.single_below > 0) for (Unit& U : units) if (!U.seqs.empty() && U.seqs.size() < (size_t)hp.single_below) { uint32_t mx = 1; for (uint32_t r : U.seqs) mx = std::max<uint32_t>(mx, (uint32_t)(RD.h_off[r + 1] - RD.h_off[r])); U.single_maxlen = mx; }
    std::vector<int> nobb;
    htc.mark("units");
    rc = run_hierarchy(ctx, d_seqs.p, RD.maxlen, nullptr, nobb, units, hp); if (rc) return rc;
    htc.mark("hierarchy");
    uint64_t total = 0; bool overflow = false; cons_off[0] = 0;
    for (uint64_t g = 0; g < n_groups; ++g) {
        const std::string& s = units[g].result;
        if (total + s.size() <= cons_cap && cons) { memcpy(cons + total, s.data(), s.size()); if (cov && units[g].cov.size() == s.size() && !s.empty()) memcpy(cov + total, units[g].cov.data(), 4 * s.size()); else if (cov) for (size_t x = 0; x < s.size(); ++x) cov[total + x] = 0; }
        else if (s.size()) overflow = true;
        total += s.size(); cons_off[g + 1] = total;
    }
    if (needed) *needed = total;
    if (overflow) NGSID_FAIL(ctx, NGSID_ERR_CAPACITY, "consensus buffer too small: need %llu bytes", (unsigned long long)total);
    return NGSID_OK;
}

namespace {

__global__ __launch_bounds__(256)
void k_strand(const uint64_t* __restrict__ mzoff , const uint32_t* __restrict__ mzcnt, const uint32_t* __restrict__ hlen, const uint64_t* __restrict__ mzcode, int k,
              const uint32_t* __restrict__ rgroup, const uint64_t* __restrict__ bcodes, const uint64_t* __restrict__ boff , uint32_t G,
              uint64_t n, uint8_t* __restrict__ orient)
{
    const int lane = threadIdx.x & 63;
    const uint64_t r = (uint64_t)blockIdx.x * (blockDim.x >> 6) + (threadIdx.x >> 6);
    if (r >= n) return;
    const uint32_t g = rgroup[r];
    if (g == 0xffffffffu) { if (lane == 0) orient[r] = 255; return; }
    const uint32_t M = hlen[r] >= (uint32_t)k ? mzcnt[r] : 0;
    const uint64_t* cf = bcodes + boff[g]; const uint32_t nf = (uint32_t)(boff[g + 1] - boff[g]);
    const uint64_t* cr = bcodes + boff[G + g]; const uint32_t nr = (uint32_t)(boff[G + g + 1] - boff[G + g]);
    int a = 0, b = 0;
    for (uint32_t x = lane; x < M; x += 64) {
        const uint64_t code = mzcode[mzoff[r] + x];
        uint32_t lo = 0, hi = nf; while (lo < hi) { const uint32_t mid = (lo + hi) >> 1; if (cf[mid] < code) lo = mid + 1; else hi = mid; }
        a += (lo < nf && cf[lo] == code);
        lo = 0; hi = nr; while (lo < hi) { const uint32_t mid = (lo + hi) >> 1; if (cr[mid] < code) lo = mid + 1; else hi = mid; }
        b += (lo < nr && cr[lo] == code);
    }
#pragma unroll
    for (int d = 32; d >= 1; d >>= 1) { a += __shfl_xor(a, d); b += __shfl_xor(b, d); }
    if (lane == 0) orient[r] = (a == 0 && b == 0) ? 255 : (b > a ? 1 : 0);
}

__host__ __device__ __forceinline__ int polish_nwin(int Bl, int W) { const int raw = Bl <= W ? 1 : (Bl + W - 1) / W; const int tail = Bl - (raw - 1) * W; return (raw >= 2 && tail < W / 10) ? raw - 1 : raw; }
__host__ __device__ __forceinline__ int polish_wlen(int Bl, int W, int w) { return w == polish_nwin(Bl, W) - 1 ? Bl - w * W : W; }

__device__ __forceinline__ uint8_t comp_base(uint8_t c) { switch (c) { case 'A': return 'T'; case 'C': return 'G'; case 'G': return 'C'; case 'T': return 'A'; default: return 'N'; } }

__global__ void k_orient(const uint8_t* __restrict__ seq, const uint8_t* __restrict__ qual, const uint64_t* __restrict__ off, uint64_t n,
                         const uint8_t* __restrict__ orient, uint8_t* __restrict__ oseq, uint8_t* __restrict__ oqual)
{
    const uint64_t r = blockIdx.x;
    if (r >= n) return;
    const uint64_t b = off[r]; const int len = (int)(off[r + 1] - b); const bool rc = orient[r] == 1;
    for (int i = threadIdx.x; i < len; i += blockDim.x) {
        if (rc) { oseq[b + i] = comp_base(seq[b + len - 1 - i]); if (qual) oqual[b + i] = qual[b + len - 1 - i]; }
        else { oseq[b + i] = seq[b + i]; if (qual) oqual[b + i] = qual[b + i]; }
    }
}

__global__ __launch_bounds__(256) void k_layers(const uint8_t* __restrict__ oseq, const uint8_t* __restrict__ oqual, const uint64_t* __restrict__ off,
                         const uint32_t* __restrict__ pair_read, const uint32_t* __restrict__ pair_group, uint64_t npairs, int nwinmax,
                         const int32_t* __restrict__ bp, const int32_t* __restrict__ span, const int32_t* __restrict__ blen ,
                         int W, double qthr, double ethr, int sub ,
                         PSeq* __restrict__ lay, uint16_t* __restrict__ valid , int* __restrict__ maxlen_out)
{
    const int lane = threadIdx.x & 63;
    const uint64_t t = (uint64_t)blockIdx.x * (blockDim.x >> 6) + (threadIdx.x >> 6);
    if (t >= npairs * (uint64_t)nwinmax) return;
    const uint64_t p = t / nwinmax; const int wdx = (int)(t % nwinmax);
    if (lane == 0) valid[t] = 0;
    const int qb = span[p * 4 + 0], qe = span[p * 4 + 1], tb = span[p * 4 + 2], te = span[p * 4 + 3];
    if (qb < 0) return;
    const int qs = qe - qb + 1, ts = te - tb + 1; const int mn = qs < ts ? qs : ts, mx = qs < ts ? ts : qs;
    if (1.0 - (double)mn / (double)mx > ethr) return;
    const int Bl = blen[pair_group[p]]; const int nw = polish_nwin(Bl, W);
    if (wdx >= nw) return;
    const int32_t* b = bp + (p * (uint64_t)nwinmax + wdx) * 4;
    int qf = b[0], ql = b[1], tf = b[2], tl = b[3];
    if (wdx == nw - 1 && wdx + 1 < nwinmax && (Bl + W - 1) / W > nw) {
        const int32_t* b2 = b + 4;
        if (b2[0] >= 0) { if (qf < 0) { qf = b2[0]; tf = b2[2]; } ql = b2[1]; tl = b2[3]; }
    }
    if (qf < 0) return;
    const int len = ql - qf + 1; if ((double)len < 0.02 * (double)W) return;
    const uint32_t read = pair_read[p]; const uint64_t rb = off[read];
    if (oqual) {
        long long sq = 0;
        for (int x = qf + lane; x <= ql; x += 64) sq += (long long)oqual[rb + x] - 33;
#pragma unroll
        for (int d = 32; d >= 1; d >>= 1) sq += __shfl_xor(sq, d);
        if ((double)sq / (double)len < qthr) return;
    }
    const int ws = wdx * W; const int wlen = polish_wlen(Bl, W, wdx);
    const int begin = tf - ws, end = tl - ws; const int offset = (int)(0.01 * (double)wlen);
    PSeq S; S.s = oseq + rb + qf; S.q = oqual ? oqual + rb + qf : nullptr; S.len = len; S.uw = 1; S.cw = 1; S.a0 = begin; S.a1 = end;
    S.mode = (begin < offset && end > wlen - offset) ? NGSID_POA_GLOBAL : (sub ? POA_MODE_SUBGRAPH : NGSID_POA_SEMI);
    if (lane == 0) { lay[t] = S; valid[t] = (uint16_t)((begin < 0 ? 0 : (begin > 65533 ? 65533 : begin)) + 1); if (len > __atomic_load_n(maxlen_out, __ATOMIC_RELAXED)) atomicMax(maxlen_out, len); }
}

std::string revcomp(const std::string& s) { std::string r(s.size(), 'N'); for (size_t i = 0; i < s.size(); ++i) { char c = s[s.size() - 1 - i]; r[i] = c == 'A' ? 'T' : c == 'C' ? 'G' : c == 'G' ? 'C' : c == 'T' ? 'A' : 'N'; } return r; }

}

struct PolishTrace { std::vector<std::string> seq; std::vector<uint64_t> used;
                     int32_t* aln = nullptr; };

static int32_t polish_impl(ngsid_ctx* ctx, const ngsid_reads_t* backbones, const ngsid_reads_t* reads, const uint32_t* read_order,
                           const uint64_t* grp_off, uint64_t n_groups, const ngsid_polish_params_t* prm,
                           uint64_t* out_off, uint8_t* out, uint64_t out_cap, uint64_t* needed, uint64_t* n_used, PolishTrace* trace);

extern "C" int32_t ngsid_polish(ngsid_ctx* ctx, const ngsid_reads_t* backbones, const ngsid_reads_t* reads, const uint32_t* read_order,
                                const uint64_t* grp_off, uint64_t n_groups, const ngsid_polish_params_t* prm,
                                uint64_t* out_off, uint8_t* out, uint64_t out_cap, uint64_t* needed, uint64_t* n_used)
{
    ApiClock api_clock_(ctx, "polish");
    return polish_impl(ctx, backbones, reads, read_order, grp_off, n_groups, prm, out_off, out, out_cap, needed, n_used, nullptr);
}

static int32_t polish_trace_impl(ngsid_ctx* ctx, const ngsid_reads_t* backbones, const ngsid_reads_t* reads, const uint32_t* read_order,
                                 const uint64_t* grp_off, uint64_t n_groups, const ngsid_polish_params_t* prm,
                                 uint64_t* it_off, uint8_t* it_out, uint64_t it_cap, uint64_t* needed, uint64_t* it_used, int32_t* it_aln)
{
    if (!ctx) return NGSID_ERR_ARG;
    if (!prm || !it_off || prm->iters < 1) NGSID_FAIL(ctx, NGSID_ERR_ARG, "ngsid_polish_trace: null argument or iters < 1");
    PolishTrace tr; tr.aln = it_aln; std::vector<uint64_t> ooff(n_groups + 1, 0); uint64_t need1 = 0;
    const int32_t rc = polish_impl(ctx, backbones, reads, read_order, grp_off, n_groups, prm, ooff.data(), nullptr, 0, &need1, nullptr, &tr);
    if (rc != NGSID_OK) return rc;
    if (tr.seq.size() != (size_t)prm->iters * n_groups || tr.used.size() != tr.seq.size()) NGSID_FAIL(ctx, NGSID_ERR_HIP, "internal: polish trace holds %zu entries for %d x %llu", tr.seq.size(), (int)prm->iters, (unsigned long long)n_groups);
    uint64_t total = 0; bool ovf = false; it_off[0] = 0;
    for (size_t x = 0; x < tr.seq.size(); ++x) {
        if (it_out && total + tr.seq[x].size() <= it_cap) memcpy(it_out + total, tr.seq[x].data(), tr.seq[x].size()); else if (tr.seq[x].size()) ovf = true;
        total += tr.seq[x].size(); it_off[x + 1] = total; if (it_used) it_used[x] = tr.used[x];
    }
    if (needed) *needed = total;
    if (ovf) NGSID_FAIL(ctx, NGSID_ERR_CAPACITY, "trace buffer too small: need %llu bytes", (unsigned long long)total);
    return NGSID_OK;
}
extern "C" int32_t ngsid_polish_trace(ngsid_ctx* ctx, const ngsid_reads_t* backbones, const ngsid_reads_t* reads, const uint32_t* read_order,
                                      const uint64_t* grp_off, uint64_t n_groups, const ngsid_polish_params_t* prm,
                                      uint64_t* it_off, uint8_t* it_out, uint64_t it_cap, uint64_t* needed, uint64_t* it_used)
{
    ApiClock api_clock_(ctx, "polish_trace");
    return polish_trace_impl(ctx, backbones, reads, read_order, grp_off, n_groups, prm, it_off, it_out, it_cap, needed, it_used, nullptr);
}
extern "C" int32_t ngsid_polish_trace_aln(ngsid_ctx* ctx, const ngsid_reads_t* backbones, const ngsid_reads_t* reads, const uint32_t* read_order,
                                          const uint64_t* grp_off, uint64_t n_groups, const ngsid_polish_params_t* prm,
                                          uint64_t* it_off, uint8_t* it_out, uint64_t it_cap, uint64_t* needed, uint64_t* it_used, int32_t* it_aln)
{
    ApiClock api_clock_(ctx, "polish_trace");
    if (ctx && !it_aln) NGSID_FAIL(ctx, NGSID_ERR_ARG, "ngsid_polish_trace_aln: null alignment buffer");
    return polish_trace_impl(ctx, backbones, reads, read_order, grp_off, n_groups, prm, it_off, it_out, it_cap, needed, it_used, it_aln);
}

int32_t ngsid_polish_orient(ngsid_ctx* ctx, const DevReads& RD, const std::vector<std::string>& B, const std::vector<uint32_t>& h_rgroup, int k, int w, OrientBufs& S, PinVec<uint8_t>& h_orient)
{
    const uint64_t N = RD.n; const uint32_t G = (uint32_t)B.size(); int32_t rc;
    DevBuf<uint64_t>& mzcode = ctx->pol_mzcode; DevBuf<uint32_t>& mzcnt = ctx->mzc_cnt; DevBuf<uint32_t>& hlen = ctx->mzc_hlen; DevBuf<uint32_t>& d_rgroup = S.d_rgroup; DevBuf<double>& herr = S.herr; DevBuf<double>& rawerr = S.rawerr; DevBuf<uint8_t>& d_orient = S.d_orient;
    HIPCHK(ctx, mzcnt.reserve(N)); HIPCHK(ctx, hlen.reserve(N));
    HIPCHK(ctx, d_rgroup.alloc(N)); HIPCHK(ctx, d_orient.alloc(N));
    HIPCHK(ctx, hipMemcpyAsync(d_rgroup.p, h_rgroup.data(), 4 * N, hipMemcpyHostToDevice, ctx->stream));
    const int sk = std::min(k, 21), sw = std::max(w, sk);
    {
        bool hit = false;
        if (ctx->mzc.valid && ctx->mzc.n == N && ctx->mzc.total == RD.total && ctx->mzc.k == sk && ctx->mzc.w == sw) {
            unsigned long long fp = 0; rc = ngsid_reads_fingerprint(ctx, RD, &fp); if (rc) return rc;
            hit = fp == ctx->mzc.fp;
        }
        if (!hit) {
            ctx->mzc.valid = false;
            HIPCHK(ctx, herr.alloc(N)); HIPCHK(ctx, rawerr.alloc(N));
            static thread_local PinVec<uint32_t> h_c, h_l; h_c.resize(N); h_l.resize(N); long long bad = -1;
            rc = ngsid_minimizers_csr(ctx, RD, sk, sw, ngsid_ctx_mz(ctx), mzcnt.p, hlen.p, herr.p, rawerr.p, h_c.data(), h_l.data(), &bad); if (rc) return rc;
            if (bad >= 0) NGSID_FAIL(ctx, NGSID_ERR_ALPHABET, "base outside ACGTN in a read (read %lld)", bad);
            if (N >= 1024) { unsigned long long fp = 0; rc = ngsid_reads_fingerprint(ctx, RD, &fp); if (rc) return rc; ctx->mzc.n = N; ctx->mzc.total = RD.total; ctx->mzc.k = sk; ctx->mzc.w = sw; ctx->mzc.fp = fp; ctx->mzc.valid = true; }
        }
    }
    {
        std::vector<std::string> two; for (uint32_t g = 0; g < G; ++g) two.push_back(B[g]); for (uint32_t g = 0; g < G; ++g) two.push_back(revcomp(B[g]));
        std::vector<uint64_t> toff(2 * G + 1, 0); std::string cat; for (size_t i = 0; i < two.size(); ++i) { cat += two[i]; toff[i + 1] = cat.size(); }
        ngsid_reads_t br{(const uint8_t*)cat.data(), nullptr, toff.data(), 2ull * G, NGSID_MEM_HOST, 0};
        DevReads BR; rc = ngsid_upload_reads(ctx, &br, &BR, false); if (rc) return rc;
        DevBuf<uint64_t> bc, boff_; DevBuf<uint32_t> bp_, bcnt, bhl; DevBuf<double> be, bw; static thread_local PinVec<uint64_t> hmo; static thread_local PinVec<uint32_t> hcnt, hhl; hcnt.resize(2 * G); hhl.resize(2 * G);
        HIPCHK(ctx, bcnt.alloc(2 * G)); HIPCHK(ctx, bhl.alloc(2 * G)); HIPCHK(ctx, be.alloc(2 * G)); HIPCHK(ctx, bw.alloc(2 * G));
        long long bad = -1;
        rc = ngsid_minimizers_csr(ctx, BR, sk, sw, MzOut{&bc, &bp_, &boff_, &hmo}, bcnt.p, bhl.p, be.p, bw.p, hcnt.data(), hhl.data(), &bad); if (rc) return rc;
        if (bad >= 0) NGSID_FAIL(ctx, NGSID_ERR_ALPHABET, "base outside ACGTN in a backbone");
        const uint64_t btot = hmo[2 * G];
        std::vector<uint64_t> hc(btot + 1);
        if (btot) HIPCHK(ctx, hipMemcpyAsync(hc.data(), bc.p, 8 * btot, hipMemcpyDeviceToHost, ctx->stream));
        HIPCHK(ctx, hipStreamSynchronize(ctx->stream));
        std::vector<uint64_t> lists, loff(2 * G + 1, 0);
        for (uint32_t i = 0; i < 2 * G; ++i) {
            const uint32_t c = hhl[i] >= (uint32_t)sk ? hcnt[i] : 0;
            std::vector<uint64_t> v(hc.begin() + hmo[i], hc.begin() + hmo[i] + c); std::sort(v.begin(), v.end());
            lists.insert(lists.end(), v.begin(), v.end()); loff[i + 1] = lists.size();
        }
        DevBuf<uint64_t> d_lists, d_loff; HIPCHK(ctx, d_lists.alloc(lists.size() + 1)); HIPCHK(ctx, d_loff.alloc(loff.size()));
        if (!lists.empty()) HIPCHK(ctx, hipMemcpyAsync(d_lists.p, lists.data(), 8 * lists.size(), hipMemcpyHostToDevice, ctx->stream));
        HIPCHK(ctx, hipMemcpyAsync(d_loff.p, loff.data(), 8 * loff.size(), hipMemcpyHostToDevice, ctx->stream));
        { ProfScope ps_(ctx, "k_strand"); hipLaunchKernelGGL(k_strand, dim3((unsigned)((N + 3) / 4)), dim3(256), 0, ctx->stream, ctx->mz_off.p, mzcnt.p, hlen.p, mzcode.p, sk, d_rgroup.p, d_lists.p, d_loff.p, G, N, d_orient.p); }
        HIPCHK(ctx, hipGetLastError());
        HIPCHK(ctx, hipStreamSynchronize(ctx->stream));
    }
    h_orient.resize(N);
    HIPCHK(ctx, hipMemcpyAsync(h_orient.data(), d_orient.p, N, hipMemcpyDeviceToHost, ctx->stream)); HIPCHK(ctx, hipStreamSynchronize(ctx->stream));
    DevBuf<uint8_t>& oseq = ctx->pol_oseq; DevBuf<uint8_t>& oqual = ctx->pol_oqual; HIPCHK(ctx, oseq.reserve(RD.total + 16)); if (RD.qual) HIPCHK(ctx, oqual.reserve(RD.total + 16));
    { ProfScope ps_(ctx, "k_orient"); hipLaunchKernelGGL(k_orient, dim3((unsigned)N), dim3(128), 0, ctx->stream, RD.seq, RD.qual, RD.off, N, d_orient.p, oseq.p, RD.qual ? oqual.p : nullptr); }
    HIPCHK(ctx, hipGetLastError());
    return NGSID_OK;
}

static int32_t polish_impl(ngsid_ctx* ctx, const ngsid_reads_t* backbones, const ngsid_reads_t* reads, const uint32_t* read_order,
                           const uint64_t* grp_off, uint64_t n_groups, const ngsid_polish_params_t* prm,
                           uint64_t* out_off, uint8_t* out, uint64_t out_cap, uint64_t* needed, uint64_t* n_used, PolishTrace* trace)
{
    if (!ctx) return NGSID_ERR_ARG;
    if (!backbones || !reads || !grp_off || !prm || !out_off) NGSID_FAIL(ctx, NGSID_ERR_ARG, "null argument");
    if (backbones->n != n_groups) NGSID_FAIL(ctx, NGSID_ERR_ARG, "one backbone per group expected");
    HostTimer ht(ctx->stream, "polish");
    DevReads RD; int32_t rc = ngsid_upload_reads(ctx, reads, &RD, false); if (rc) return rc;
    if (!read_order && grp_off[n_groups] > RD.n) NGSID_FAIL(ctx, NGSID_ERR_ARG, "group offsets exceed the read set");
    if (read_order) for (uint64_t x = 0; x < grp_off[n_groups]; ++x) if (read_order[x] >= RD.n) NGSID_FAIL(ctx, NGSID_ERR_ARG, "read_order[%llu] out of range", (unsigned long long)x);
    const uint64_t N = RD.n; const uint32_t G = (uint32_t)n_groups;
    const int W = prm->window > 0 ? prm->window : 500;
    ht.mark("upload + checks");
    std::vector<std::string> B(G);
    {
        std::vector<uint64_t> boff(G + 1); std::vector<uint8_t> bseq;
        if (backbones->mem == NGSID_MEM_DEVICE) {
            HIPCHK(ctx, hipMemcpy(boff.data(), backbones->off, 8 * (G + 1), hipMemcpyDeviceToHost)); bseq.resize(boff[G] + 1);
            if (boff[G]) HIPCHK(ctx, hipMemcpy(bseq.data(), backbones->seq, boff[G], hipMemcpyDeviceToHost));
        } else { memcpy(boff.data(), backbones->off, 8 * (G + 1)); bseq.assign(backbones->seq, backbones->seq + boff[G]); bseq.push_back(0); }
        for (uint32_t g = 0; g < G; ++g) B[g].assign((const char*)bseq.data() + boff[g], (size_t)(boff[g + 1] - boff[g]));
    }
    if (N == 0 || G == 0) {
        uint64_t total = 0; out_off[0] = 0; bool ovf = false;
        for (uint32_t g = 0; g < G; ++g) { if (trace) {} else if (total + B[g].size() <= out_cap && out) memcpy(out + total, B[g].data(), B[g].size()); else if (B[g].size()) ovf = true; total += B[g].size(); out_off[g + 1] = total; if (n_used) n_used[g] = 0; }
        if (trace) for (int it = 0; it < prm->iters; ++it) for (uint32_t g = 0; g < G; ++g) { trace->seq.push_back(B[g]); trace->used.push_back(0); }
        if (trace && trace->aln) for (uint64_t x = 0; x < (uint64_t)prm->iters * grp_off[n_groups] * 6; ++x) trace->aln[x] = -1;
        if (needed) *needed = total; if (ovf) NGSID_FAIL(ctx, NGSID_ERR_CAPACITY, "output buffer too small"); return NGSID_OK;
    }
    std::vector<uint32_t> h_rgroup(N, 0xffffffffu); std::vector<uint8_t> tgs(G, 0);
    for (uint32_t g = 0; g < G; ++g) {
        double tot = 0; const uint64_t ns = grp_off[g + 1] - grp_off[g];
        for (uint64_t x = grp_off[g]; x < grp_off[g + 1]; ++x) {
            const uint64_t r = read_order ? read_order[x] : x;
            if (h_rgroup[r] != 0xffffffffu) NGSID_FAIL(ctx, NGSID_ERR_ARG, "read %llu is listed twice (groups %u and %u): strand and layers are kept per read, list every read under one backbone", (unsigned long long)r, h_rgroup[r], g);
            h_rgroup[r] = g; tot += (double)(RD.h_off[r + 1] - RD.h_off[r]);
        }
        tgs[g] = ns > 0 && (tot / (double)ns) > 1000.0;
    }
    ht.mark("group map");
    OrientBufs ob; DevBuf<int> flag; HIPCHK(ctx, flag.alloc(1)); static thread_local PinVec<uint8_t> h_orient;
    rc = ngsid_polish_orient(ctx, RD, B, h_rgroup, prm->k, prm->w, ob, h_orient); if (rc) return rc;
    DevBuf<uint8_t>& oseq = ctx->pol_oseq; DevBuf<uint8_t>& oqual = ctx->pol_oqual;
    ht.mark("minimizers + strand + orient");
    static thread_local PinVec<uint32_t> pair_read, pair_group; pair_read.clear(); pair_group.clear();
    const bool want_aln = trace && trace->aln; const uint64_t NL = grp_off[n_groups];
    std::vector<uint64_t> pair_pos;
    for (uint64_t x = 0; x < grp_off[n_groups]; ++x) { const uint64_t r = read_order ? read_order[x] : x; if (h_orient[r] != 255) { pair_read.push_back((uint32_t)r); pair_group.push_back(h_rgroup[r]); if (want_aln) pair_pos.push_back(x); } }
    DevBuf<int32_t> d_dist; static thread_local PinVec<int32_t> h_span, h_dist;
    if (want_aln) { HIPCHK(ctx, d_dist.alloc(pair_read.size() + 1)); h_span.resize(pair_read.size() * 4 + 4); h_dist.resize(pair_read.size() + 1); }
    uint64_t NP = pair_read.size();
    DevBuf<uint32_t> d_pair_read, d_pair_group; DevBuf<int32_t> d_open, d_span, d_blen; DevBuf<int32_t>& d_bp = ctx->pol_bp; DevBuf<uint8_t>& d_lay_raw = ctx->pol_lay; DevBuf<uint16_t>& d_valid = ctx->pol_valid;
    HIPCHK(ctx, d_pair_read.alloc(NP)); HIPCHK(ctx, d_pair_group.alloc(NP)); HIPCHK(ctx, d_open.alloc(NP)); HIPCHK(ctx, d_span.alloc(NP * 4)); HIPCHK(ctx, d_blen.alloc(G));
    if (NP) { HIPCHK(ctx, hipMemcpyAsync(d_pair_read.p, pair_read.data(), 4 * NP, hipMemcpyHostToDevice, ctx->stream)); HIPCHK(ctx, hipMemcpyAsync(d_pair_group.p, pair_group.data(), 4 * NP, hipMemcpyHostToDevice, ctx->stream));
              HIPCHK(ctx, hipMemsetD32Async((hipDeviceptr_t)d_open.p, prm->aln_open, NP, ctx->stream)); }
    HIPCHK(ctx, hipStreamSynchronize(ctx->stream));
    std::vector<uint64_t> used(G, 0);
    ht.mark("orient + pairs");

    std::vector<uint8_t> stable(G, 0);
    for (int it = 0; it < prm->iters; ++it) {
        if (prm->stop_when_stable && it > 0) {
            bool any_active = false; for (uint32_t g = 0; g < G; ++g) any_active = any_active || !stable[g];
            if (!any_active) break;
            size_t keep = 0;
            for (size_t p = 0; p < pair_read.size(); ++p) if (!stable[pair_group[p]]) { pair_read[keep] = pair_read[p]; pair_group[keep] = pair_group[p]; if (want_aln) pair_pos[keep] = pair_pos[p]; ++keep; }
            if (keep != pair_read.size()) {
                pair_read.resize(keep); pair_group.resize(keep); NP = keep; if (want_aln) pair_pos.resize(keep);
                if (NP) { HIPCHK(ctx, hipMemcpyAsync(d_pair_read.p, pair_read.data(), 4 * NP, hipMemcpyHostToDevice, ctx->stream)); HIPCHK(ctx, hipMemcpyAsync(d_pair_group.p, pair_group.data(), 4 * NP, hipMemcpyHostToDevice, ctx->stream)); HIPCHK(ctx, hipStreamSynchronize(ctx->stream)); }
            }
        }
        std::vector<uint64_t> boff(G + 1, 0); std::string cat; std::vector<int32_t> blen(G); int nwinmax = 1; uint32_t maxb = 0;
        for (uint32_t g = 0; g < G; ++g) { cat += B[g]; boff[g + 1] = cat.size(); blen[g] = (int32_t)B[g].size(); nwinmax = std::max(nwinmax, (int)((B[g].size() + W - 1) / W)); maxb = std::max<uint32_t>(maxb, (uint32_t)B[g].size()); }
        ngsid_reads_t br{(const uint8_t*)cat.data(), nullptr, boff.data(), G, NGSID_MEM_HOST, 0};
        DevReads BB; rc = ngsid_upload_reads(ctx, &br, &BB, false); if (rc) return rc;
        HIPCHK(ctx, hipMemcpyAsync(d_blen.p, blen.data(), 4 * G, hipMemcpyHostToDevice, ctx->stream));
        for (uint32_t g = 0; g < G; ++g) if (!stable[g]) used[g] = 0;
        std::vector<Unit> units; std::vector<PSeq> bbs; std::vector<int> bb_len; std::vector<std::pair<uint32_t, int>> unit_gw;
        static thread_local PinVec<uint16_t> h_valid; int max_layer = 1;
        HIPCHK(ctx, hipMemsetAsync(flag.p, 0, sizeof(int), ctx->stream));
        if (NP) {
            HIPCHK(ctx, d_bp.reserve(NP * (uint64_t)nwinmax * 4)); HIPCHK(ctx, d_lay_raw.reserve(sizeof(PSeq) * NP * (uint64_t)nwinmax)); HIPCHK(ctx, d_valid.reserve(NP * (uint64_t)nwinmax));
            AlignJob J{};
            J.qseq = oseq.p; J.qoff = RD.off; J.tseq = BB.seq; J.toff = BB.off; J.qidx = d_pair_read.p; J.tidx = d_pair_group.p; J.npairs = NP;
            J.match = prm->aln_match; J.mismatch = prm->aln_mismatch; J.ext = prm->aln_ext; J.k = 1; J.open = d_open.p; J.match_id = nullptr;
            J.score = nullptr; J.ncols = nullptr; J.nmatch = nullptr; J.region = nullptr; J.bp = d_bp.p; J.bp_windows = nwinmax; J.window = W; J.span = d_span.p;
            int aln_mode = prm->aln_mode & ~NGSID_ALN_SUBGRAPH; if (aln_mode == 2) aln_mode = 1;
            if (aln_mode == 3) { aln_mode = 1; J.clip = 1; }
            if (aln_mode == 1) rc = ngsid_launch_ed_align(ctx, J, RD.maxlen, maxb, want_aln ? d_dist.p : nullptr);
            else rc = ngsid_launch_align(ctx, J, RD.maxlen, maxb, prm->aln_open);
            if (rc) return rc;
            const uint64_t T = NP * (uint64_t)nwinmax;
            { ProfScope ps_(ctx, "k_layers"); hipLaunchKernelGGL(k_layers, dim3((unsigned)((T + 3) / 4)), dim3(256), 0, ctx->stream, oseq.p, RD.qual ? oqual.p : nullptr, RD.off, d_pair_read.p, d_pair_group.p, NP, nwinmax,
                               d_bp.p, d_span.p, d_blen.p, W, prm->quality_threshold, prm->error_threshold, (prm->aln_mode & NGSID_ALN_SUBGRAPH) ? 1 : 0, (PSeq*)d_lay_raw.p, d_valid.p, flag.p); }
            HIPCHK(ctx, hipGetLastError());
            h_valid.resize(T);
            HIPCHK(ctx, hipMemcpyAsync(&max_layer, flag.p, 4, hipMemcpyDeviceToHost, ctx->stream));
            HIPCHK(ctx, hipMemcpyAsync(h_valid.data(), d_valid.p, 2 * T, hipMemcpyDeviceToHost, ctx->stream));
            if (want_aln) { HIPCHK(ctx, hipMemcpyAsync(h_span.data(), d_span.p, 16 * NP, hipMemcpyDeviceToHost, ctx->stream)); if (aln_mode == 1) HIPCHK(ctx, hipMemcpyAsync(h_dist.data(), d_dist.p, 4 * NP, hipMemcpyDeviceToHost, ctx->stream)); }
            HIPCHK(ctx, hipStreamSynchronize(ctx->stream));
            if (want_aln) {
                int32_t* A = trace->aln + (size_t)it * NL * 6;
                if (it == 0) for (uint64_t x = 0; x < NL * 6; ++x) A[x] = -1; else memcpy(A, A - NL * 6, sizeof(int32_t) * NL * 6);
                for (uint64_t p = 0; p < NP; ++p) {
                    int32_t* a = A + pair_pos[p] * 6; const uint32_t r = pair_read[p]; const int32_t ql = (int32_t)(RD.h_off[r + 1] - RD.h_off[r]);
                    const int32_t qf = h_span[p * 4], qe = h_span[p * 4 + 1], tf = h_span[p * 4 + 2], te = h_span[p * 4 + 3];
                    if (qf < 0) { for (int c = 0; c < 6; ++c) a[c] = -1; continue; }
                    const bool rcs = h_orient[r] == 1;
                    a[0] = rcs ? 1 : 0; a[1] = rcs ? ql - 1 - qe : qf; a[2] = rcs ? ql - qf : qe + 1; a[3] = tf; a[4] = te + 1; a[5] = aln_mode == 1 ? h_dist[p] : -1;
                }
            }
        } else if (want_aln) { int32_t* A = trace->aln + (size_t)it * NL * 6; if (it == 0) for (uint64_t x = 0; x < NL * 6; ++x) A[x] = -1; else memcpy(A, A - NL * 6, sizeof(int32_t) * NL * 6); }
        ht.mark("align + layers + valid copy");
        std::vector<std::vector<int>> unit_of(G);
        for (uint32_t g = 0; g < G; ++g) { if (stable[g]) continue; const int nw = polish_nwin((int)B[g].size(), W); unit_of[g].assign(nw, -1);
            for (int wdx = 0; wdx < nw; ++wdx) { unit_of[g][wdx] = (int)units.size(); units.emplace_back(); unit_gw.push_back({g, wdx}); } }
        {
            std::vector<uint32_t> ubase(G), unw(G), npg(G, 0);
            for (uint32_t g = 0; g < G; ++g) { unw[g] = (uint32_t)unit_of[g].size(); ubase[g] = unw[g] ? (uint32_t)unit_of[g][0] : 0; }
            for (uint64_t p = 0; p < NP; ++p) npg[pair_group[p]]++;
            const uint32_t* pg = pair_group.data(); const uint16_t* hv0 = h_valid.data();
            bool by_group = true; std::vector<uint64_t> gbeg(G + 1, 0);
            for (uint64_t p = 1; p < NP; ++p) if (pg[p] < pg[p - 1]) { by_group = false; break; }
            if (by_group) { uint64_t acc = 0; for (uint32_t g = 0; g < G; ++g) { gbeg[g] = acc; acc += npg[g]; } gbeg[G] = acc; }
            auto order_unit = [&](std::vector<uint32_t>& v, std::vector<uint32_t>& tmpv, std::vector<uint32_t>& cnt) {
                if (v.size() < 2) return;
                uint32_t kmax = 0; bool sorted = true;
                for (size_t x = 0; x < v.size(); ++x) { const uint32_t kx = hv0[v[x]]; kmax = std::max(kmax, kx); if (x && hv0[v[x - 1]] > kx) sorted = false; }
                if (sorted) return;
                cnt.assign((size_t)kmax + 2, 0);
                for (uint32_t id : v) cnt[hv0[id] + 1]++;
                for (size_t k2 = 1; k2 < cnt.size(); ++k2) cnt[k2] += cnt[k2 - 1];
                tmpv.resize(v.size());
                for (uint32_t id : v) tmpv[cnt[hv0[id]]++] = id;
                std::copy(tmpv.begin(), tmpv.end(), v.begin());
            };
            if (by_group && NP >= 65536) {
                std::vector<uint64_t> used_g(G, 0);
                const unsigned hw = std::max(1u, std::min(16u, std::thread::hardware_concurrency()));
                const size_t ntask = units.size() + G;
                std::atomic<size_t> next_task{0};
                auto worker = [&]() {
                    std::vector<uint32_t> tmpv, cnt;
                    for (;;) {
                        const size_t t = next_task.fetch_add(1); if (t >= ntask) break;
                        if (t < units.size()) {
                            const uint32_t g = unit_gw[t].first, wdx = (uint32_t)unit_gw[t].second;
                            auto& v = units[t].seqs; v.resize(npg[g]); uint32_t* c = v.data();
                            for (uint64_t p = gbeg[g]; p < gbeg[g + 1]; ++p) { *c = (uint32_t)(p * (uint64_t)nwinmax + wdx); c += hv0[p * (uint64_t)nwinmax + wdx] != 0; }
                            v.resize((size_t)(c - v.data()));
                            order_unit(v, tmpv, cnt);
                        } else {
                            const uint32_t g = (uint32_t)(t - units.size()); const uint32_t nwg = unw[g]; uint64_t u = 0;
                            for (uint64_t p = gbeg[g]; p < gbeg[g + 1]; ++p) { const uint16_t* hv = hv0 + p * (uint64_t)nwinmax; uint32_t any = 0; for (uint32_t wdx = 0; wdx < nwg; ++wdx) any |= hv[wdx] != 0; u += any; }
                            used_g[g] = u;
                        }
                    }
                };
                std::vector<std::thread> th; for (unsigned x = 1; x < hw; ++x) th.emplace_back(worker);
                worker(); for (auto& t : th) t.join();
                for (uint32_t g = 0; g < G; ++g) used[g] += (uint32_t)used_g[g];
            } else {
                std::vector<uint32_t*> cur(units.size(), nullptr);
                for (uint32_t g = 0; g < G; ++g) for (uint32_t wdx = 0; wdx < unw[g]; ++wdx) { auto& v = units[ubase[g] + wdx].seqs; v.resize(npg[g]); cur[ubase[g] + wdx] = v.data(); }
                for (uint64_t p = 0; p < NP; ++p) {
                    const uint32_t g = pg[p]; const uint16_t* hv = hv0 + p * (uint64_t)nwinmax; const uint32_t nwg = unw[g], ub = ubase[g]; uint32_t any = 0;
                    for (uint32_t wdx = 0; wdx < nwg; ++wdx) { const uint32_t v = hv[wdx] != 0; *cur[ub + wdx] = (uint32_t)(p * (uint64_t)nwinmax + wdx); cur[ub + wdx] += v; any |= v; }
                    used[g] += any;
                }
                for (size_t u = 0; u < units.size(); ++u) if (cur[u]) units[u].seqs.resize((size_t)(cur[u] - units[u].seqs.data()));
                std::vector<uint32_t> tmpv, cnt;
                for (size_t u = 0; u < units.size(); ++u) order_unit(units[u].seqs, tmpv, cnt);
            }
        }
        std::vector<size_t> nlayers(units.size());
        for (size_t u = 0; u < units.size(); ++u) {
            nlayers[u] = units[u].seqs.size();
            if (units[u].seqs.size() < 2) { units[u].seqs.clear(); units[u].done = true; continue; }
            const uint32_t g = unit_gw[u].first; const int ws = unit_gw[u].second * W; const int wlen = polish_wlen((int)B[g].size(), W, unit_gw[u].second);
            PSeq S; S.s = BB.seq + boff[g] + ws; S.q = nullptr; S.len = wlen; S.uw = 0; S.cw = 0; S.mode = NGSID_POA_GLOBAL; S.a0 = 0; S.a1 = -1;
            units[u].bb = (int)bbs.size(); bbs.push_back(S); bb_len.push_back(wlen);
        }
        DevBuf<PSeq> d_bbs; HIPCHK(ctx, d_bbs.alloc(bbs.size()));
        if (!bbs.empty()) HIPCHK(ctx, hipMemcpyAsync(d_bbs.p, bbs.data(), sizeof(PSeq) * bbs.size(), hipMemcpyHostToDevice, ctx->stream));
        bool any_tgs = prm->trim == 2; for (uint32_t g = 0; g < G; ++g) any_tgs = any_tgs || (tgs[g] && prm->trim);
        HierParams hp{prm->match, prm->mismatch, prm->gap, prm->band > 0 ? prm->band : (RD.maxlen <= NGSID_POA_BAND64_MAXLEN ? 64 : 128), prm->node_cap, prm->tile_depth, NGSID_POA_GLOBAL, any_tgs, (prm->trim >= 2 ? 1 : 0) | (prm->trim == 3 ? 4 : 0)};
        hp.single_below = prm->single_below > 0 ? prm->single_below : 0;
        hp.sub = (prm->aln_mode & NGSID_ALN_SUBGRAPH) != 0;
        if (hp.single_below > 0) for (size_t u = 0; u < units.size(); ++u) {
            Unit& U = units[u]; if (U.done || U.seqs.size() >= (size_t)hp.single_below) continue;
            uint32_t mx = (uint32_t)std::max(1, bb_len[U.bb]);
            for (uint32_t id : U.seqs) { const uint32_t r = pair_read[id / (uint32_t)nwinmax]; mx = std::max<uint32_t>(mx, (uint32_t)(RD.h_off[r + 1] - RD.h_off[r])); }
            U.single_maxlen = mx;
        }
        ht.mark("unit lists");
        rc = run_hierarchy(ctx, (const PSeq*)d_lay_raw.p, (uint32_t)std::max(max_layer, 1), d_bbs.p, bb_len, units, hp); if (rc) return rc;
        ht.mark("hierarchy");
        std::vector<std::string> NB(G);
        for (size_t u = 0; u < units.size(); ++u) {
            const uint32_t g = unit_gw[u].first; const int ws = unit_gw[u].second * W; const int wlen = polish_wlen((int)B[g].size(), W, unit_gw[u].second);
            std::string c = units[u].has_result ? units[u].result : std::string();
            if (!c.empty() && prm->trim && (tgs[g] || prm->trim == 2) && units[u].cov.size() == c.size()) {
                const uint32_t avg = (uint32_t)(nlayers[u] / 2); int b = 0, e = (int)c.size() - 1;
                for (; b < (int)c.size(); ++b) if (units[u].cov[b] >= avg) break;
                for (; e >= 0; --e) if (units[u].cov[e] >= avg) break;
                if (b < e) c = c.substr(b, e - b + 1);
            }
            if (c.empty()) c = B[g].substr(ws, wlen);
            NB[g] += c;
        }
        for (uint32_t g = 0; g < G; ++g) { if (stable[g]) NB[g] = B[g]; else if (prm->stop_when_stable && NB[g] == B[g]) stable[g] = 1; }
        B.swap(NB);
        if (trace) for (uint32_t g = 0; g < G; ++g) { trace->seq.push_back(B[g]); trace->used.push_back(used[g]); }
    }
    if (trace && trace->aln) for (size_t it = trace->seq.size() / std::max<uint32_t>(G, 1); it < (size_t)prm->iters; ++it) { if (it == 0) { for (uint64_t x = 0; x < grp_off[n_groups] * 6; ++x) trace->aln[x] = -1; } else memcpy(trace->aln + it * grp_off[n_groups] * 6, trace->aln + (it - 1) * grp_off[n_groups] * 6, sizeof(int32_t) * grp_off[n_groups] * 6); }
    if (trace) while (trace->seq.size() < (size_t)prm->iters * G) { const size_t x = trace->seq.size() - G; trace->seq.push_back(trace->seq[x]); trace->used.push_back(trace->used[x]); }
    uint64_t total = 0; bool ovf = false; out_off[0] = 0;
    for (uint32_t g = 0; g < G; ++g) {
        if (trace) {  }
        else if (total + B[g].size() <= out_cap && out) memcpy(out + total, B[g].data(), B[g].size()); else if (B[g].size()) ovf = true;
        total += B[g].size(); out_off[g + 1] = total; if (n_used) n_used[g] = used[g];
    }
    if (needed) *needed = total;
    if (ovf) NGSID_FAIL(ctx, NGSID_ERR_CAPACITY, "output buffer too small: need %llu bytes", (unsigned long long)total);
    return NGSID_OK;
}
```

Measured before the change: 1.469 million.

## Build POA unit sequence lists on device via radix sort instead of host

```diff
diff --git a/ngspeciesid_amd/csrc/k_poa.h b/ngspeciesid_amd/csrc/k_poa.h
--- a/ngspeciesid_amd/csrc/k_poa.h
+++ b/ngspeciesid_amd/csrc/k_poa.h
@@ -20,3 +20,8 @@
 int32_t poa_check_limits(ngsid_ctx* ctx, const PoaPlan& P, int m, int g);
 int32_t poa_prepare(ngsid_ctx* ctx, PoaPlan& P, uint32_t max_jobs, int m, int g);
 int32_t poa_launch(ngsid_ctx* ctx, const PoaPlan& P, PoaJobSet J, int band, bool redo, uint32_t* work_ctr, bool sub = false);
+
+struct PoaListBufs { DevBuf<uint64_t> key_in, key_out; DevBuf<uint32_t> slot_in, list, rec; DevBuf<uint8_t> tmp; DevBuf<int32_t> ginfo ; };
+static inline size_t poa_list_rec_words(uint32_t G, uint32_t U) { return 2ull * U + 2 + G; }
+int32_t poa_polish_unit_lists(ngsid_ctx* ctx, PoaListBufs& B, const uint16_t* valid, const uint32_t* pair_group, const uint32_t* pair_read, const uint64_t* read_off,
+                              uint64_t npairs, int nwinmax, uint32_t G, uint32_t U, int single_below);
diff --git a/ngspeciesid_amd/csrc/k_poa_lists.hip b/ngspeciesid_amd/csrc/k_poa_lists.hip
--- /dev/null
+++ b/ngspeciesid_amd/csrc/k_poa_lists.hip
@@ -0,0 +1,71 @@
+#include "ngsid_internal.h"
+#include "k_poa.h"
+#include <hipcub/hipcub.hpp>
+
+namespace {
+
+__global__ __launch_bounds__(256) void k_poa_unit_keys(const uint16_t* __restrict__ valid, const uint32_t* __restrict__ pair_group, uint64_t npairs, int nwinmax,
+                                                      const int32_t* __restrict__ ginfo, uint32_t G, uint32_t U, uint64_t* __restrict__ key, uint32_t* __restrict__ slot, uint32_t* __restrict__ used)
+{
+    const int lane = threadIdx.x & 63;
+    const uint64_t p = (uint64_t)blockIdx.x * blockDim.x + threadIdx.x;
+    const bool active = p < npairs;
+    const uint32_t g = active ? pair_group[p] : 0xffffffffu;
+    bool any = false;
+    if (active) {
+        const int ub = g < G ? ginfo[g] : -1, nw = g < G ? ginfo[G + g] : 0;
+        for (int wdx = 0; wdx < nwinmax; ++wdx) {
+            const uint64_t t = p * (uint64_t)nwinmax + wdx; const uint32_t v = valid[t];
+            const bool ok = ub >= 0 && wdx < nw && v != 0;
+            key[t] = ok ? ((uint64_t)(uint32_t)(ub + wdx) << 16) | v : (uint64_t)U << 16;
+            slot[t] = (uint32_t)t; any = any || ok;
+        }
+    }
+    unsigned long long rest = __ballot(active);
+    while (rest) {
+        const int leader = __ffsll((long long)rest) - 1;
+        const uint32_t gl = __shfl(g, leader);
+        const unsigned long long same = __ballot(active && g == gl), cnt = __ballot(active && g == gl && any);
+        if (lane == leader && cnt && gl < G) atomicAdd(&used[gl], (uint32_t)__popcll(cnt));
+        rest &= ~same;
+    }
+}
+
+__global__ __launch_bounds__(256) void k_poa_unit_bounds(const uint64_t* __restrict__ key, uint32_t T, uint32_t U, int single_below, const uint32_t* __restrict__ list, int nwinmax,
+                                                        const uint32_t* __restrict__ pair_read, const uint64_t* __restrict__ read_off, uint32_t* __restrict__ unit_off, uint32_t* __restrict__ unit_maxread)
+{
+    const uint32_t u = blockIdx.x * blockDim.x + threadIdx.x;
+    if (u > U) return;
+    auto first_of = [&](uint32_t unit) { const uint64_t k = (uint64_t)unit << 16; uint32_t lo = 0, hi = T; while (lo < hi) { const uint32_t mid = lo + ((hi - lo) >> 1); if (key[mid] < k) lo = mid + 1; else hi = mid; } return lo; };
+    const uint32_t a = first_of(u);
+    unit_off[u] = a;
+    if (u == U) return;
+    uint32_t mx = 0;
+    if (single_below > 0) {
+        const uint32_t n = first_of(u + 1) - a;
+        if (n >= 2 && n < (uint32_t)single_below) for (uint32_t x = 0; x < n; ++x) { const uint32_t r = pair_read[list[a + x] / (uint32_t)nwinmax]; const uint32_t len = (uint32_t)(read_off[r + 1] - read_off[r]); mx = len > mx ? len : mx; }
+    }
+    unit_maxread[u] = mx;
+}
+
+}
+
+int32_t poa_polish_unit_lists(ngsid_ctx* ctx, PoaListBufs& B, const uint16_t* valid, const uint32_t* pair_group, const uint32_t* pair_read, const uint64_t* read_off,
+                              uint64_t npairs, int nwinmax, uint32_t G, uint32_t U, int single_below)
+{
+    const uint64_t T64 = npairs * (uint64_t)nwinmax;
+    if (T64 == 0 || T64 >= (1ull << 31)) NGSID_FAIL(ctx, NGSID_ERR_ARG, "internal: %llu layer slots cannot be listed on the device", (unsigned long long)T64);
+    const uint32_t T = (uint32_t)T64;
+    HIPCHK(ctx, B.key_in.reserve(T)); HIPCHK(ctx, B.key_out.reserve(T)); HIPCHK(ctx, B.slot_in.reserve(T)); HIPCHK(ctx, B.list.reserve(T));
+    uint32_t* rec = B.rec.p;
+    { ProfScope ps_(ctx, "k_poa_unit_keys"); hipLaunchKernelGGL(k_poa_unit_keys, dim3((unsigned)((npairs + 255) / 256)), dim3(256), 0, ctx->stream, valid, pair_group, npairs, nwinmax, B.ginfo.p, G, U, B.key_in.p, B.slot_in.p, rec + U + 2); }
+    HIPCHK(ctx, hipGetLastError());
+    int end_bit = 17; while (end_bit < 48 && (1ull << (end_bit - 16)) <= (uint64_t)U) ++end_bit;
+    size_t tb = 0;
+    HIPCHK(ctx, hipcub::DeviceRadixSort::SortPairs(nullptr, tb, B.key_in.p, B.key_out.p, B.slot_in.p, B.list.p, (int)T, 0, end_bit, ctx->stream));
+    HIPCHK(ctx, B.tmp.reserve(tb + 16));
+    { ProfScope ps_(ctx, "poa_unit_sort"); HIPCHK(ctx, hipcub::DeviceRadixSort::SortPairs(B.tmp.p, tb, B.key_in.p, B.key_out.p, B.slot_in.p, B.list.p, (int)T, 0, end_bit, ctx->stream)); }
+    { ProfScope ps_(ctx, "k_poa_unit_bounds"); hipLaunchKernelGGL(k_poa_unit_bounds, dim3((U + 1 + 255) / 256), dim3(256), 0, ctx->stream, B.key_out.p, T, U, single_below, B.list.p, nwinmax, pair_read, read_off, rec + 1, rec + U + 2 + G); }
+    HIPCHK(ctx, hipGetLastError());
+    return NGSID_OK;
+}
diff --git a/ngspeciesid_amd/csrc/ngsid_api.hip b/ngspeciesid_amd/csrc/ngsid_api.hip
--- a/ngspeciesid_amd/csrc/ngsid_api.hip
+++ b/ngspeciesid_amd/csrc/ngsid_api.hip
@@ -572,7 +572,7 @@
 extern "C" int32_t ngsid_ctx_option(ngsid_ctx* ctx, const char* name, int64_t value)
 {
     if (!ctx || !name) return NGSID_ERR_ARG;
-    static const char* known[] = {"minimizers_chunk_bases", "poa_level_budget_mb", "cluster_block", "cluster_block_cap", "cluster_trunc", "cluster_seg_order", "ed_band", "ed_win_all", "align32", "align_noclass", "poa_tiles_per_cu", "minimizers_lean", "minimizers_mode", "poa_host_levels", "align_paired", "poa_out_slots", "ed_lds_pad_kb", "ed_win6", "support_budget_mb", "demux_chunk_reads"};
+    static const char* known[] = {"minimizers_chunk_bases", "poa_level_budget_mb", "cluster_block", "cluster_block_cap", "cluster_trunc", "cluster_seg_order", "ed_band", "ed_win_all", "align32", "align_noclass", "poa_tiles_per_cu", "minimizers_lean", "minimizers_mode", "poa_host_levels", "device_unit_lists", "align_paired", "poa_out_slots", "ed_lds_pad_kb", "ed_win6", "support_budget_mb", "demux_chunk_reads"};
     for (const char* k : known) if (!strcmp(k, name)) { ctx->options[name] = (long long)value; return NGSID_OK; }
     if (!strcmp(name, "touch")) {
         if (ctx->mzc_fp.n < 2) HIPCHK(ctx, ctx->mzc_fp.alloc(2));
diff --git a/ngspeciesid_amd/csrc/poa_host.hip b/ngspeciesid_amd/csrc/poa_host.hip
--- a/ngspeciesid_amd/csrc/poa_host.hip
+++ b/ngspeciesid_amd/csrc/poa_host.hip
@@ -12,6 +12,8 @@
 
 struct Unit {
     std::vector<uint32_t> seqs;
+    uint32_t dev_n = 0, dev_off = 0;
+    size_t nseq() const { return dev_n ? dev_n : seqs.size(); }
     int bb = -1;
     bool done = false;
     uint32_t single_maxlen = 0;
@@ -41,7 +43,8 @@
     out[i] = S;
 }
 
-struct HierParams { int m, n, g, band, node_cap, D, upper_mode; bool want_cov; int trim_tiles; int single_below = 0; bool sub = false; };
+struct HierParams { int m, n, g, band, node_cap, D, upper_mode; bool want_cov; int trim_tiles; int single_below = 0; bool sub = false;
+                    bool dev_lists = false; const uint32_t* list0 = nullptr; };
 
 struct TileLists {
     PinVec<uint32_t> job_off, seq_idx, job_unit; PinVec<int32_t> job_bb; PinVec<uint8_t> job_final ;
@@ -71,6 +74,25 @@
         }
         if (unit_rec) { unit_rec[u] = ncur; unit_rec[nu + u] = job0; unit_rec[2 * nu + u] = T.njobs() - job0; }
     }
+}
+uint32_t plan_tiles(TileLists& T, std::vector<Unit>& units, const std::vector<int>& bb_len, int D, uint32_t* unit_rec, uint32_t* nseq)
+{
+    T.maxD = 0; T.maxn = 0; T.maxbb = 0; T.any_nobb = false;
+    const size_t nu = units.size(); uint32_t njobs = 0, ns = 0;
+    for (size_t u = 0; u < nu; ++u) {
+        Unit& U = units[u];
+        const uint32_t ncur = U.done ? 0u : (uint32_t)U.nseq(), nt = poa_ntiles(ncur, D > 0 ? (uint32_t)D : ncur);
+        if (ncur == 0) U.done = true;
+        else {
+            T.maxD = std::max(T.maxD, nt == 1 ? ncur : std::max((uint32_t)D, ncur - (nt - 1) * (uint32_t)D));
+            if (U.bb >= 0) T.maxbb = std::max(T.maxbb, bb_len[U.bb]); else T.any_nobb = true;
+            T.maxn = std::max(T.maxn, ncur);
+        }
+        unit_rec[u] = ncur; unit_rec[nu + u] = njobs; unit_rec[2 * nu + u] = nt; unit_rec[3 * nu + u] = ns; unit_rec[4 * nu + u] = U.dev_off;
+        njobs += nt; ns += ncur;
+    }
+    *nseq = ns;
+    return njobs;
 }
 int32_t upload_tiles(ngsid_ctx* ctx, const TileLists& T, ngsid_ctx::PoaLevelBufs& B, bool final_, bool unit)
 {
@@ -380,6 +402,15 @@
     }
 }
 
+__global__ __launch_bounds__(256) void k_poa_gather_seq0(HierDev H, const uint32_t* __restrict__ src, const uint32_t* __restrict__ src_off, uint32_t nseq, uint32_t* __restrict__ seq_idx)
+{
+    for (uint32_t i = blockIdx.x * blockDim.x + threadIdx.x; i < nseq; i += gridDim.x * blockDim.x) {
+        uint32_t lo = 0, hi = H.U;
+        while (hi - lo > 1) { const uint32_t mid = (lo + hi) >> 1; if (H.unit_seq0[mid] <= i) lo = mid; else hi = mid; }
+        const uint32_t x = src_off[lo] + (i - H.unit_seq0[lo]);
+        seq_idx[i] = src ? src[x] : x;
+    }
+}
 
 int32_t run_hierarchy_dev(ngsid_ctx* ctx, const PSeq* d_level0, uint32_t maxlen0, const PSeq* d_bbs, const std::vector<int>& bb_len,
                           std::vector<Unit>& units, const HierParams& hp, bool* done)
@@ -390,10 +421,11 @@
     const uint32_t U = (uint32_t)units.size();
     HostTimer ht(ctx->stream, "hierarchy (device levels)");
     static thread_local TileLists T; static thread_local PinVec<uint32_t> u_u32; static thread_local PinVec<int32_t> u_i32;
-    u_u32.assign(3ull * U, 0); u_i32.assign(3ull * U, 0);
-    build_tiles(T, units, bb_len, hp.D, u_u32.data());
+    u_u32.assign(5ull * U, 0); u_i32.assign(3ull * U, 0);
+    uint32_t njobs_dl = 0, nseq_dl = 0;
+    if (hp.dev_lists) njobs_dl = plan_tiles(T, units, bb_len, hp.D, u_u32.data(), &nseq_dl); else build_tiles(T, units, bb_len, hp.D, u_u32.data());
     for (uint32_t u = 0; u < U; ++u) { const int bb = units[u].bb; u_i32[u] = bb; u_i32[U + u] = bb >= 0 ? bb_len[bb] : 0; u_i32[2ull * U + u] = -2; }
-    const uint32_t njobs0 = T.njobs(), maxD = T.maxD; const uint64_t maxn = T.maxn;
+    const uint32_t njobs0 = hp.dev_lists ? njobs_dl : T.njobs(), maxD = T.maxD; const uint64_t maxn = T.maxn;
     if (njobs0 == 0) return NGSID_OK;
     const int Lb = std::max<int>((int)maxlen0, T.maxbb), Lb2 = Lb + Lb / 4 + 16;
     PoaPlan plan = poa_plan(hp, std::max(T.maxbb, T.any_nobb ? Lb2 : 1), (uint32_t)Lb2, hp.sub);
@@ -429,9 +461,17 @@
     HIPCHK(ctx, hipMemcpyAsync(H.unit_job0[0], u_u32.data() + U, 4ull * U, hipMemcpyHostToDevice, ctx->stream));
     HIPCHK(ctx, hipMemcpyAsync(H.unit_njobs[0], u_u32.data() + 2ull * U, 4ull * U, hipMemcpyHostToDevice, ctx->stream));
     HIPCHK(ctx, hipMemcpyAsync(d_i32.p, u_i32.data(), 12ull * U, hipMemcpyHostToDevice, ctx->stream));
-    { int32_t rc = upload_tiles(ctx, T, ctx->poa_lv[0], hp.trim_tiles & 4, true); if (rc) return rc; }
-    static thread_local PinVec<uint32_t> h_nj; h_nj.assign(1, njobs0);
-    HIPCHK(ctx, hipMemcpyAsync(d_ctrl.p + C_NJOBS, h_nj.data(), 4, hipMemcpyHostToDevice, ctx->stream));
+    static thread_local PinVec<uint32_t> h_nj; h_nj.assign(3, 0); h_nj[0] = njobs0; h_nj[C_NSEQ - C_NJOBS] = nseq_dl;
+    HIPCHK(ctx, hipMemcpyAsync(d_ctrl.p + C_NJOBS, h_nj.data(), 12, hipMemcpyHostToDevice, ctx->stream));
+    DevBuf<uint32_t> d_src_off;
+    if (hp.dev_lists) {
+        HIPCHK(ctx, d_src_off.alloc(U)); HIPCHK(ctx, ctx->poa_lv[0].seq_idx.reserve(nseq_dl));
+        HIPCHK(ctx, hipMemcpyAsync(H.unit_seq0, u_u32.data() + 3ull * U, 4ull * U, hipMemcpyHostToDevice, ctx->stream));
+        HIPCHK(ctx, hipMemcpyAsync(d_src_off.p, u_u32.data() + 4ull * U, 4ull * U, hipMemcpyHostToDevice, ctx->stream));
+        hipLaunchKernelGGL(k_poa_gather_seq0, dim3(std::min<uint32_t>((nseq_dl + 255) / 256, 4096u)), dim3(256), 0, ctx->stream, H, hp.list0, d_src_off.p, nseq_dl, ctx->poa_lv[0].seq_idx.p);
+        hipLaunchKernelGGL(k_poa_fill_jobs, dim3(std::min<uint32_t>((njobs0 + 255) / 256, 1024u)), dim3(256), 0, ctx->stream, H, L[0], 1);
+        HIPCHK(ctx, hipGetLastError());
+    } else { int32_t rc = upload_tiles(ctx, T, ctx->poa_lv[0], hp.trim_tiles & 4, true); if (rc) return rc; }
     ht.mark("L0 lists + upload");
     static thread_local PinVec<uint32_t> h_ctrl; h_ctrl.resize(C_WORDS);
     int level = 0;
@@ -491,7 +531,17 @@
     bool done = false;
     int32_t rc = run_hierarchy_dev(ctx, d_level0, maxlen0, d_bbs, bb_len, units, hp, &done);
     if (rc || done) return rc;
-    return run_hierarchy_host(ctx, d_level0, maxlen0, d_bbs, bb_len, units, hp);
+    if (!hp.dev_lists) return run_hierarchy_host(ctx, d_level0, maxlen0, d_bbs, bb_len, units, hp);
+    HIPCHK(ctx, hipStreamSynchronize(ctx->stream));
+    for (Unit& U : units) {
+        if (U.done || !U.dev_n) continue;
+        U.seqs.resize(U.dev_n);
+        if (hp.list0) HIPCHK(ctx, hipMemcpy(U.seqs.data(), hp.list0 + U.dev_off, 4ull * U.dev_n, hipMemcpyDeviceToHost));
+        else for (uint32_t x = 0; x < U.dev_n; ++x) U.seqs[x] = U.dev_off + x;
+        U.dev_n = 0;
+    }
+    HierParams hh = hp; hh.dev_lists = false; hh.list0 = nullptr;
+    return run_hierarchy_host(ctx, d_level0, maxlen0, d_bbs, bb_len, units, hh);
 }
 
 int32_t run_hierarchy(ngsid_ctx* ctx, const PSeq* d_level0, uint32_t maxlen0, const PSeq* d_bbs, const std::vector<int>& bb_len,
@@ -530,7 +580,7 @@
     const double per_tile = (double)slots * ((double)capV * (need_cov ? 5.0 : 1.0) + 64.0) * (hp.D > 0 ? 1.0 + 1.25 * (double)slots / (double)hp.D : 1.0) + 32.0;
     std::vector<std::pair<size_t, size_t>> batches; size_t b0 = 0; double acc = 0;
     for (size_t u = 0; u < units.size(); ++u) {
-        const uint32_t ncur = units[u].done ? 0u : (uint32_t)units[u].seqs.size();
+        const uint32_t ncur = units[u].done ? 0u : (uint32_t)units[u].nseq();
         const double need = ncur ? per_tile * (double)poa_ntiles(ncur, hp.D > 0 ? (uint32_t)hp.D : ncur) : 0.0;
         if (u > b0 && acc + need > (double)budget) { batches.push_back({b0, u}); b0 = u; acc = 0; }
         acc += need;
@@ -589,13 +639,26 @@
     if (RD.n) hipLaunchKernelGGL(k_make_pseq_reads, dim3((unsigned)((RD.n + 255) / 256)), dim3(256), 0, ctx->stream, RD.seq, RD.qual, RD.off, RD.n, prm->mode, weight ? d_weight.p : (const uint32_t*)nullptr, d_seqs.p);
     HIPCHK(ctx, hipGetLastError());
     std::vector<Unit> units(n_groups);
-    for (uint64_t g = 0; g < n_groups; ++g) {
+    const bool dev_lists = ngsid_opt(ctx, "device_unit_lists", 1) != 0 && grp_off[n_groups] < (1ull << 32);
+    DevBuf<uint32_t> d_order; static thread_local PinVec<uint32_t> h_order;
+    if (dev_lists) {
+        for (uint64_t g = 0; g < n_groups; ++g) { units[g].dev_off = (uint32_t)grp_off[g]; units[g].dev_n = (uint32_t)(grp_off[g + 1] - grp_off[g]); }
+        if (read_order && grp_off[n_groups]) {
+            h_order.assign(read_order, read_order + grp_off[n_groups]);
+            HIPCHK(ctx, d_order.alloc(h_order.size())); HIPCHK(ctx, hipMemcpyAsync(d_order.p, h_order.data(), 4 * h_order.size(), hipMemcpyHostToDevice, ctx->stream));
+        }
+    } else for (uint64_t g = 0; g < n_groups; ++g) {
         if (read_order) units[g].seqs.assign(read_order + grp_off[g], read_order + grp_off[g + 1]);
         else { units[g].seqs.resize(grp_off[g + 1] - grp_off[g]); for (uint64_t r = grp_off[g]; r < grp_off[g + 1]; ++r) units[g].seqs[r - grp_off[g]] = (uint32_t)r; }
     }
     HierParams hp{prm->match, prm->mismatch, prm->gap, prm->band > 0 ? prm->band : (RD.maxlen <= NGSID_POA_BAND64_MAXLEN ? 64 : 128), prm->node_cap, prm->tile_depth, prm->mode, cov != nullptr, prm->trim > 0 ? 1 : 0};
     hp.single_below = prm->single_below > 0 ? prm->single_below : 0;
-    if (hp.single_below > 0) for (Unit& U : units) if (!U.seqs.empty() && U.seqs.size() < (size_t)hp.single_below) { uint32_t mx = 1; for (uint32_t r : U.seqs) mx = std::max<uint32_t>(mx, (uint32_t)(RD.h_off[r + 1] - RD.h_off[r])); U.single_maxlen = mx; }
+    hp.dev_lists = dev_lists; hp.list0 = dev_lists && read_order ? d_order.p : nullptr;
+    if (hp.single_below > 0) for (uint64_t g = 0; g < n_groups; ++g) {
+        const uint64_t ng = grp_off[g + 1] - grp_off[g]; if (ng == 0 || ng >= (uint64_t)hp.single_below) continue;
+        uint32_t mx = 1; for (uint64_t x = grp_off[g]; x < grp_off[g + 1]; ++x) { const uint64_t r = read_order ? read_order[x] : x; mx = std::max<uint32_t>(mx, (uint32_t)(RD.h_off[r + 1] - RD.h_off[r])); }
+        units[g].single_maxlen = mx;
+    }
     std::vector<int> nobb;
     htc.mark("units");
     rc = run_hierarchy(ctx, d_seqs.p, RD.maxlen, nullptr, nobb, units, hp); if (rc) return rc;
@@ -870,6 +933,8 @@
     ht.mark("orient + pairs");
 
     std::vector<uint8_t> stable(G, 0);
+    PoaListBufs LB; static thread_local PinVec<uint32_t> h_rec; static thread_local PinVec<int32_t> h_ginfo;
+    const int single_below = prm->single_below > 0 ? prm->single_below : 0;
     for (int it = 0; it < prm->iters; ++it) {
         if (prm->stop_when_stable && it > 0) {
             bool any_active = false; for (uint32_t g = 0; g < G; ++g) any_active = any_active || !stable[g];
@@ -889,7 +954,32 @@
         for (uint32_t g = 0; g < G; ++g) if (!stable[g]) used[g] = 0;
         std::vector<Unit> units; std::vector<PSeq> bbs; std::vector<int> bb_len; std::vector<std::pair<uint32_t, int>> unit_gw;
         static thread_local PinVec<uint16_t> h_valid; int max_layer = 1;
-        HIPCHK(ctx, hipMemsetAsync(flag.p, 0, sizeof(int), ctx->stream));
+        std::vector<std::vector<int>> unit_of(G);
+        for (uint32_t g = 0; g < G; ++g) { if (stable[g]) continue; const int nw = polish_nwin((int)B[g].size(), W); unit_of[g].assign(nw, -1);
+            for (int wdx = 0; wdx < nw; ++wdx) { unit_of[g][wdx] = (int)units.size(); units.emplace_back(); unit_gw.push_back({g, wdx}); } }
+        const uint32_t NU = (uint32_t)units.size();
+        const bool dev_lists = NP && ngsid_opt(ctx, "device_unit_lists", 1) != 0 && NP * (uint64_t)nwinmax < (1ull << 31);
+        int* d_maxlen = flag.p;
+        if (dev_lists) {
+            const size_t words = poa_list_rec_words(G, NU);
+            HIPCHK(ctx, LB.rec.reserve(words)); HIPCHK(ctx, LB.ginfo.reserve(2ull * G)); h_rec.resize(words); h_ginfo.resize(2ull * G);
+            for (uint32_t g = 0; g < G; ++g) { h_ginfo[g] = unit_of[g].empty() ? -1 : unit_of[g][0]; h_ginfo[G + g] = (int32_t)unit_of[g].size(); }
+            HIPCHK(ctx, hipMemsetAsync(LB.rec.p, 0, 4 * words, ctx->stream));
+            HIPCHK(ctx, hipMemcpyAsync(LB.ginfo.p, h_ginfo.data(), 8ull * G, hipMemcpyHostToDevice, ctx->stream));
+            d_maxlen = (int*)LB.rec.p;
+        } else HIPCHK(ctx, hipMemsetAsync(flag.p, 0, sizeof(int), ctx->stream));
+        int aln_mode_rec = 0;
+        auto write_aln_records = [&]() {
+            int32_t* A = trace->aln + (size_t)it * NL * 6;
+            if (it == 0) for (uint64_t x = 0; x < NL * 6; ++x) A[x] = -1; else memcpy(A, A - NL * 6, sizeof(int32_t) * NL * 6);
+            for (uint64_t p = 0; p < NP; ++p) {
+                int32_t* a = A + pair_pos[p] * 6; const uint32_t r = pair_read[p]; const int32_t ql = (int32_t)(RD.h_off[r + 1] - RD.h_off[r]);
+                const int32_t qf = h_span[p * 4], qe = h_span[p * 4 + 1], tf = h_span[p * 4 + 2], te = h_span[p * 4 + 3];
+                if (qf < 0) { for (int c = 0; c < 6; ++c) a[c] = -1; continue; }
+                const bool rcs = h_orient[r] == 1;
+                a[0] = rcs ? 1 : 0; a[1] = rcs ? ql - 1 - qe : qf; a[2] = rcs ? ql - qf : qe + 1; a[3] = tf; a[4] = te + 1; a[5] = aln_mode_rec == 1 ? h_dist[p] : -1;
+            }
+        };
         if (NP) {
             HIPCHK(ctx, d_bp.reserve(NP * (uint64_t)nwinmax * 4)); HIPCHK(ctx, d_lay_raw.reserve(sizeof(PSeq) * NP * (uint64_t)nwinmax)); HIPCHK(ctx, d_valid.reserve(NP * (uint64_t)nwinmax));
             AlignJob J{};
@@ -903,30 +993,30 @@
             if (rc) return rc;
             const uint64_t T = NP * (uint64_t)nwinmax;
             { ProfScope ps_(ctx, "k_layers"); hipLaunchKernelGGL(k_layers, dim3((unsigned)((T + 3) / 4)), dim3(256), 0, ctx->stream, oseq.p, RD.qual ? oqual.p : nullptr, RD.off, d_pair_read.p, d_pair_group.p, NP, nwinmax,
-                               d_bp.p, d_span.p, d_blen.p, W, prm->quality_threshold, prm->error_threshold, (prm->aln_mode & NGSID_ALN_SUBGRAPH) ? 1 : 0, (PSeq*)d_lay_raw.p, d_valid.p, flag.p); }
+                               d_bp.p, d_span.p, d_blen.p, W, prm->quality_threshold, prm->error_threshold, (prm->aln_mode & NGSID_ALN_SUBGRAPH) ? 1 : 0, (PSeq*)d_lay_raw.p, d_valid.p, d_maxlen); }
             HIPCHK(ctx, hipGetLastError());
-            h_valid.resize(T);
-            HIPCHK(ctx, hipMemcpyAsync(&max_layer, flag.p, 4, hipMemcpyDeviceToHost, ctx->stream));
-            HIPCHK(ctx, hipMemcpyAsync(h_valid.data(), d_valid.p, 2 * T, hipMemcpyDeviceToHost, ctx->stream));
-            if (want_aln) { HIPCHK(ctx, hipMemcpyAsync(h_span.data(), d_span.p, 16 * NP, hipMemcpyDeviceToHost, ctx->stream)); if (aln_mode == 1) HIPCHK(ctx, hipMemcpyAsync(h_dist.data(), d_dist.p, 4 * NP, hipMemcpyDeviceToHost, ctx->stream)); }
-            HIPCHK(ctx, hipStreamSynchronize(ctx->stream));
-            if (want_aln) {
-                int32_t* A = trace->aln + (size_t)it * NL * 6;
-                if (it == 0) for (uint64_t x = 0; x < NL * 6; ++x) A[x] = -1; else memcpy(A, A - NL * 6, sizeof(int32_t) * NL * 6);
-                for (uint64_t p = 0; p < NP; ++p) {
-                    int32_t* a = A + pair_pos[p] * 6; const uint32_t r = pair_read[p]; const int32_t ql = (int32_t)(RD.h_off[r + 1] - RD.h_off[r]);
-                    const int32_t qf = h_span[p * 4], qe = h_span[p * 4 + 1], tf = h_span[p * 4 + 2], te = h_span[p * 4 + 3];
-                    if (qf < 0) { for (int c = 0; c < 6; ++c) a[c] = -1; continue; }
-                    const bool rcs = h_orient[r] == 1;
-                    a[0] = rcs ? 1 : 0; a[1] = rcs ? ql - 1 - qe : qf; a[2] = rcs ? ql - qf : qe + 1; a[3] = tf; a[4] = te + 1; a[5] = aln_mode == 1 ? h_dist[p] : -1;
+            aln_mode_rec = aln_mode;
+            if (dev_lists) {
+                rc = poa_polish_unit_lists(ctx, LB, d_valid.p, d_pair_group.p, d_pair_read.p, RD.off, NP, nwinmax, G, NU, single_below); if (rc) return rc;
+                HIPCHK(ctx, hipMemcpyAsync(h_rec.data(), LB.rec.p, 4 * h_rec.size(), hipMemcpyDeviceToHost, ctx->stream));
+                if (want_aln) {
+                    rc = ngsid_side_streams(ctx); if (rc) return rc;
+                    HIPCHK(ctx, hipEventRecord(ctx->ev_fork, ctx->stream)); HIPCHK(ctx, hipStreamWaitEvent(ctx->side[0], ctx->ev_fork, 0));
+                    HIPCHK(ctx, hipMemcpyAsync(h_span.data(), d_span.p, 16 * NP, hipMemcpyDeviceToHost, ctx->side[0])); if (aln_mode == 1) HIPCHK(ctx, hipMemcpyAsync(h_dist.data(), d_dist.p, 4 * NP, hipMemcpyDeviceToHost, ctx->side[0]));
                 }
+                HIPCHK(ctx, hipStreamSynchronize(ctx->stream));
+                max_layer = (int)h_rec[0];
+            } else {
+                h_valid.resize(T);
+                HIPCHK(ctx, hipMemcpyAsync(&max_layer, flag.p, 4, hipMemcpyDeviceToHost, ctx->stream));
+                HIPCHK(ctx, hipMemcpyAsync(h_valid.data(), d_valid.p, 2 * T, hipMemcpyDeviceToHost, ctx->stream));
+                if (want_aln) { HIPCHK(ctx, hipMemcpyAsync(h_span.data(), d_span.p, 16 * NP, hipMemcpyDeviceToHost, ctx->stream)); if (aln_mode == 1) HIPCHK(ctx, hipMemcpyAsync(h_dist.data(), d_dist.p, 4 * NP, hipMemcpyDeviceToHost, ctx->stream)); }
+                HIPCHK(ctx, hipStreamSynchronize(ctx->stream));
+                if (want_aln) write_aln_records();
             }
         } else if (want_aln) { int32_t* A = trace->aln + (size_t)it * NL * 6; if (it == 0) for (uint64_t x = 0; x < NL * 6; ++x) A[x] = -1; else memcpy(A, A - NL * 6, sizeof(int32_t) * NL * 6); }
         ht.mark("align + layers + valid copy");
-        std::vector<std::vector<int>> unit_of(G);
-        for (uint32_t g = 0; g < G; ++g) { if (stable[g]) continue; const int nw = polish_nwin((int)B[g].size(), W); unit_of[g].assign(nw, -1);
-            for (int wdx = 0; wdx < nw; ++wdx) { unit_of[g][wdx] = (int)units.size(); units.emplace_back(); unit_gw.push_back({g, wdx}); } }
-        {
+        if (!dev_lists) {
             std::vector<uint32_t> ubase(G), unw(G), npg(G, 0);
             for (uint32_t g = 0; g < G; ++g) { unw[g] = (uint32_t)unit_of[g].size(); ubase[g] = unw[g] ? (uint32_t)unit_of[g][0] : 0; }
             for (uint64_t p = 0; p < NP; ++p) npg[pair_group[p]]++;
@@ -984,10 +1074,14 @@
                 for (size_t u = 0; u < units.size(); ++u) order_unit(units[u].seqs, tmpv, cnt);
             }
         }
+        if (dev_lists) {
+            for (uint32_t u = 0; u < NU; ++u) { units[u].dev_off = h_rec[1 + u]; units[u].dev_n = h_rec[2 + u] - h_rec[1 + u]; }
+            for (uint32_t g = 0; g < G; ++g) if (!stable[g]) used[g] = h_rec[NU + 2 + g];
+        }
         std::vector<size_t> nlayers(units.size());
         for (size_t u = 0; u < units.size(); ++u) {
-            nlayers[u] = units[u].seqs.size();
-            if (units[u].seqs.size() < 2) { units[u].seqs.clear(); units[u].done = true; continue; }
+            nlayers[u] = units[u].nseq();
+            if (nlayers[u] < 2) { units[u].seqs.clear(); units[u].dev_n = 0; units[u].done = true; continue; }
             const uint32_t g = unit_gw[u].first; const int ws = unit_gw[u].second * W; const int wlen = polish_wlen((int)B[g].size(), W, unit_gw[u].second);
             PSeq S; S.s = BB.seq + boff[g] + ws; S.q = nullptr; S.len = wlen; S.uw = 0; S.cw = 0; S.mode = NGSID_POA_GLOBAL; S.a0 = 0; S.a1 = -1;
             units[u].bb = (int)bbs.size(); bbs.push_back(S); bb_len.push_back(wlen);
@@ -996,17 +1090,20 @@
         if (!bbs.empty()) HIPCHK(ctx, hipMemcpyAsync(d_bbs.p, bbs.data(), sizeof(PSeq) * bbs.size(), hipMemcpyHostToDevice, ctx->stream));
         bool any_tgs = prm->trim == 2; for (uint32_t g = 0; g < G; ++g) any_tgs = any_tgs || (tgs[g] && prm->trim);
         HierParams hp{prm->match, prm->mismatch, prm->gap, prm->band > 0 ? prm->band : (RD.maxlen <= NGSID_POA_BAND64_MAXLEN ? 64 : 128), prm->node_cap, prm->tile_depth, NGSID_POA_GLOBAL, any_tgs, (prm->trim >= 2 ? 1 : 0) | (prm->trim == 3 ? 4 : 0)};
-        hp.single_below = prm->single_below > 0 ? prm->single_below : 0;
+        hp.single_below = single_below;
         hp.sub = (prm->aln_mode & NGSID_ALN_SUBGRAPH) != 0;
+        hp.dev_lists = dev_lists; hp.list0 = dev_lists ? LB.list.p : nullptr;
         if (hp.single_below > 0) for (size_t u = 0; u < units.size(); ++u) {
-            Unit& U = units[u]; if (U.done || U.seqs.size() >= (size_t)hp.single_below) continue;
+            Unit& U = units[u]; if (U.done || U.nseq() >= (size_t)hp.single_below) continue;
             uint32_t mx = (uint32_t)std::max(1, bb_len[U.bb]);
+            if (dev_lists) mx = std::max(mx, h_rec[NU + 2 + G + u]);
             for (uint32_t id : U.seqs) { const uint32_t r = pair_read[id / (uint32_t)nwinmax]; mx = std::max<uint32_t>(mx, (uint32_t)(RD.h_off[r + 1] - RD.h_off[r])); }
             U.single_maxlen = mx;
         }
         ht.mark("unit lists");
         rc = run_hierarchy(ctx, (const PSeq*)d_lay_raw.p, (uint32_t)std::max(max_layer, 1), d_bbs.p, bb_len, units, hp); if (rc) return rc;
         ht.mark("hierarchy");
+        if (dev_lists && want_aln) { HIPCHK(ctx, hipStreamSynchronize(ctx->side[0])); write_aln_records(); }
         std::vector<std::string> NB(G);
         for (size_t u = 0; u < units.size(); ++u) {
             const uint32_t g = unit_gw[u].first; const int ws = unit_gw[u].second * W; const int wlen = polish_wlen((int)B[g].size(), W, unit_gw[u].second);
```

New measurement: 1.466 million. Within noise of the previous version (-0.2%).
